# Algomorph/LevelSetFusion-Python

Measured on AMD Instinct MI355X. Metric: voxel-warp-updates/sec, higher is better.
Workload: dtype f32

## Files before the change

include/lsf_hip.h:

```cpp
#ifndef LSF_HIP_H
#define LSF_HIP_H

#include <stdint.h>

#ifdef __cplusplus
extern "C" {
#endif

#define LSF_ABI_VERSION 4
#define LSF_MAX_KERNEL_TAPS 31

#define LSF_ERR_BAD_ARGUMENT (-1)
#define LSF_ERR_BAD_DIMS (-2)
#define LSF_ERR_KERNEL_TOO_LONG (-3)
#define LSF_ERR_RCCL_UNAVAILABLE (-4)
#define LSF_ERR_RCCL_FAILED (-5)
#define LSF_ERR_NOT_RESIDENT (-6)

typedef struct lsf_grid {
    int32_t dims;
    int32_t nz, ny, nx;
    int32_t z_begin, z_end;
    int32_t z_global_offset;
    int32_t y_global_offset;
// ... 83 lines not shown
    int32_t previous_max;
    int32_t reserved;
    int32_t packed_nz;
    int32_t packed_z_global_offset;
} lsf_hier_params;

int lsf_hier_iteration(const float *packed_live4, const float *canonical, float *warp_planar,
                       const float *g_prev_planar, float *g_out_planar, const lsf_grid *grid,
                       const lsf_hier_params *params, const lsf_gate *gate, lsf_iteration_record *record,
                       void *stream);

int lsf_hier_level_run_2d(const float *packed_live4, const float *canonical, float *warp_a, float *warp_b, float *g_a,
                          float *g_b, const lsf_grid *grid, const lsf_hier_params *params, const double *taps_host,
                          int32_t n_taps, lsf_iteration_record *records, int32_t iterations,
                          int32_t iterations_per_launch, float threshold, void *stream);
int lsf_hier_update(const float *g_planar, float *warp_planar, const lsf_grid *grid, float rate,
                    const lsf_gate *gate, lsf_iteration_record *record, void *stream);

#define LSF_SMOOTHING_TIKHONOV 0
#define LSF_SMOOTHING_KILLING 1
#define LSF_DATA_BASIC 0
#define LSF_DATA_THRESHOLDED_FDM 2
#define LSF_ENERGY_NONE 0
#define LSF_ENERGY_DIRECT 1
#define LSF_ENERGY_VECTORIZED 2

typedef struct lsf_slavcheva_params {
    double isomorphic_enforcement_factor_f64;
    float rate;
    float data_term_weight;
    float smoothing_term_weight;
    float level_set_term_weight;
    float isomorphic_enforcement_factor;
    float killing_c1;
    int32_t smoothing_method;
    int32_t data_method;
    int32_t level_set_enabled;
    int32_t energy_mode;
    int32_t zero_gradient_on_snap;
    int32_t reserved;
} lsf_slavcheva_params;

int lsf_slavcheva_gradient(const float *live, const float *canonical, const float *warp_prev_planar,
                           float *g_out_planar, const lsf_grid *grid, const lsf_slavcheva_params *params,
                           const lsf_gate *gate, lsf_iteration_record *record, const int32_t *band_list,
                           int64_t band_count, void *stream);

#define LSF_BAND_ALL 0
#define LSF_BAND_INTERIOR 1
#define LSF_BAND_BOUNDARY 2

int64_t lsf_band_scratch_elements(const lsf_grid *grid);
int lsf_band_count(const float *live, const float *canonical, const lsf_grid *grid, int32_t subset,
                   int32_t *scratch, int64_t *count_out, void *stream);
int lsf_band_list_fill(const float *live, const float *canonical, const lsf_grid *grid, int32_t subset,
                       const int32_t *scratch, int32_t *list, void *stream);

int64_t lsf_state_prepare_scratch_elements(const lsf_grid *grid);
int lsf_state_pack_needed(const float *live, float *state_a, float *state_b, const lsf_grid *grid, int32_t *scratch,
                          int32_t reach, int32_t invert, void *stream);

int lsf_band_list_fill_prepared(const lsf_grid *grid, int32_t subset, const int32_t *scratch, int32_t *list,
                                void *stream);
int lsf_state_prepare(const float *live, const float *canonical, float *state_a, float *state_b,
                      const lsf_grid *grid, int32_t *scratch, int64_t *counts_out, void *stream);
int lsf_state_pack(const float *live, const float *warp_planar, float *state_a, float *state_b,
                   const lsf_grid *grid, void *stream);
int lsf_state_unpack(const float *state, float *live_out, float *warp_planar_out, float *warp_interleaved_out,
                     const lsf_grid *grid, void *stream);
int64_t lsf_state_finalize_scratch_elements(const lsf_grid *grid);
int lsf_state_finalize(const float *state, const float *canonical, float *live_out, float *warp_planar_out,
                       float *warp_interleaved_out, const lsf_grid *grid, float lower_threshold,
                       double *statistics16, double *scratch, void *stream);
int lsf_planar_finalize(const float *live, const float *warp_planar, const float *canonical, float *live_out,
                        float *warp_interleaved_out, const lsf_grid *grid, float lower_threshold,
                        double *statistics16, double *scratch, void *stream);

int lsf_state_finalize_listed(const float *state, const float *canonical, float *live_out, float *warp_interleaved_out,
                              const lsf_grid *grid, const int32_t *const *band_lists, const int64_t *band_counts,
                              int32_t n_lists, int64_t opposite_count, int64_t first_opposite, float lower_threshold,
                              double *statistics16, double *scratch, const int32_t *skip_flag,
                              const lsf_iteration_record *guard_records, int32_t guard_count, float guard_limit,
                              void *stream);
int lsf_slavcheva_state_iteration(const float *state_in, const float *canonical, float *state_out,
                                  const lsf_grid *grid, const lsf_slavcheva_params *params, const lsf_gate *gate,
                                  lsf_iteration_record *record, const int32_t *band_list, int64_t band_count,
                                  int32_t band_subset, void *stream);

int lsf_cumulative_warp_compose(const float *state, const float *psi_in, float *psi_out, const lsf_grid *grid,
                                const lsf_gate *gate, const int32_t *band_list, int64_t band_count, void *stream);

typedef struct lsf_band_box {
    int32_t origin;
    int32_t reserved;
    uint64_t mask;
} lsf_band_box;
int64_t lsf_band_boxes_scratch_elements(const lsf_grid *grid);
int lsf_band_boxes_count(const lsf_grid *grid, int32_t subset, const int32_t *prepare_scratch, int32_t *box_scratch,
                         int64_t *count_out, void *stream);
int lsf_band_boxes_fill(const lsf_grid *grid, int32_t subset, const int32_t *prepare_scratch, const int32_t *box_scratch,
                        lsf_band_box *boxes, void *stream);
int lsf_band_boxes_canonical(const float *canonical, const lsf_grid *grid, const lsf_band_box *boxes, int64_t box_count,
                             float *canonical_boxed, void *stream);
int lsf_slavcheva_state_iteration_boxes(const float *state_in, const float *canonical_boxed, float *state_out,
                                        const lsf_grid *grid, const lsf_slavcheva_params *params, const lsf_gate *gate,
                                        lsf_iteration_record *record, const lsf_band_box *boxes, int64_t box_count,
                                        void *stream);

typedef struct lsf_run_loop {
    int32_t min_iterations;
    int32_t max_iterations;
    float lower_threshold, upper_threshold;
    int32_t check_interval;
    int32_t reserved;
} lsf_run_loop;
typedef struct lsf_state_run {
    const float *live;
    const float *canonical;
    float *state[2];
    int32_t *prepare_scratch;
    int64_t *totals_device;
    int64_t *totals_host;
    lsf_grid grid;
    int32_t sparse_reach;
    int32_t second_state_late;
    int32_t *box_scratch;
    int32_t box_all;
    int32_t reserved;
} lsf_state_run;
typedef struct lsf_state_run_result {
    float *max_value;
    int64_t *argmax;
    double *energies3;
    uint8_t *executed;
    int32_t final_state;
    int32_t n_lists;
    int32_t reach_exceeded;
    int32_t compact_faces;
} lsf_state_run_result;
int lsf_state_run_begin(const lsf_state_run *run, void *stream);
int lsf_state_run_finish(const lsf_state_run *run, const lsf_slavcheva_params *params, int32_t *list_interior,
                         int32_t *list_boundary, lsf_band_box *boxes, float *box_canonical, lsf_iteration_record *records,
                         int32_t iterations, const lsf_run_loop *loop ,
                         float *live_out,
                         float lower_threshold, double *statistics16, double *finalize_scratch, int64_t *words_device,
                         int64_t *words_host, lsf_state_run_result *result, void *stream);
int lsf_state_run_finish_rows(const lsf_state_run *run, const lsf_slavcheva_params *params, int32_t *list_interior,
                              int32_t *list_boundary, lsf_band_box *boxes, float *box_canonical,
                              lsf_iteration_record *records, int32_t iterations, const lsf_run_loop *loop, float *live_out,
                              float lower_threshold, double *statistics16, double *finalize_scratch, int64_t *words_device,
                              int64_t *words_host, lsf_state_run_result *result, int64_t *record_rows,
                              int64_t record_rows_elements, int32_t *rows_taken, void *stream);
int64_t lsf_state_run_rows_elements(const lsf_grid *grid, int32_t iterations, int32_t n_lists);

int lsf_sobolev_run_finish(const lsf_state_run *run, const lsf_slavcheva_params *params, const double *taps_host,
                           int32_t n_taps, int32_t *list_interior, int32_t *list_boundary, int32_t *list_all,
                           lsf_band_box *boxes, float *g4_a, float *g4_b, lsf_iteration_record *records, int32_t iterations,
                           const lsf_run_loop *loop, float *live_out, float lower_threshold, double *statistics16,
                           double *finalize_scratch, int64_t *words_device, int64_t *words_host,
                           lsf_state_run_result *result, void *stream);

int lsf_sobolev_state_gradient(const float *state, const float *canonical, float *g_raw4, const lsf_grid *grid,
                               const lsf_slavcheva_params *params, const lsf_gate *gate, lsf_iteration_record *record,
                               const int32_t *band_list, int64_t band_count, void *stream);
int lsf_sobolev_state_gradient_x(const float *state, const float *canonical, float *out4, const lsf_grid *grid,
                                 const lsf_slavcheva_params *params, const double *taps_host, int32_t n_taps,
                                 const lsf_gate *gate, lsf_iteration_record *record, const int32_t *band_list,
                                 int64_t band_count, int32_t out_bricks, void *stream);
int lsf_zero_listed4(float *field4, const lsf_grid *grid, const int32_t *band_list, int64_t band_count, int32_t bricks,
                     void *stream);
int lsf_convolve_axis_listed4(const float *in4, float *out4, const float *zero_mask_source4, const lsf_grid *grid,
                              int32_t axis, const double *taps_host, int32_t n_taps, const lsf_gate *gate,
                              const int32_t *band_list, int64_t band_count, void *stream);
int lsf_band_list_strip_major(const int32_t *band_list, int64_t band_count, const lsf_grid *grid, int32_t strips,
                              int32_t *out, int32_t *scratch, void *stream);
int lsf_sobolev_state_update(const float *in4, const float *zero_mask_source4, const float *state_in, float *state_out,
                             float *g_out4, const lsf_grid *grid, const lsf_slavcheva_params *params, int32_t axis,
                             const double *taps_host, int32_t n_taps, const lsf_gate *gate,
                             lsf_iteration_record *record, const int32_t *band_list, int64_t band_count,
                             int32_t first_list, void *stream);
int lsf_sobolev_state_update_boxes(const float *in4, const float *state_in, float *state_out, float *g_out4,
                                   const lsf_grid *grid, const lsf_slavcheva_params *params, const double *taps_host,
                                   int32_t n_taps, const lsf_gate *gate, lsf_iteration_record *record,
                                   const lsf_band_box *boxes, int64_t box_count, void *stream);

#define LSF_SLAB_LAUNCH 0
#define LSF_SLAB_EXCHANGE 1
#define LSF_SLAB_EXCHANGE_DEFERRED 2
#define LSF_SLAB_RESUME 3
typedef struct lsf_slab_comm lsf_slab_comm;
typedef struct lsf_slab_layout {
    int32_t nz, ny, nx;
    int32_t z_begin, z_end;
    int32_t halo;
    int32_t lo_rank, hi_rank;
} lsf_slab_layout;
typedef struct lsf_slab_part {
    lsf_grid grid;
    const int32_t *band_list[2];
    int64_t band_count[2];
    int32_t band_subset[2];
    int32_t n_lists;
    int32_t reserved;
} lsf_slab_part;
typedef struct lsf_slab_faces {
    const int32_t *send_list[2], *recv_list[2];
    float *send_msg[2], *recv_msg[2];
    int64_t send_count[2], recv_count[2];
} lsf_slab_faces;
int lsf_merge_sorted_runs(const int32_t *const *a, const int64_t *n_a, const int32_t *const *b, const int64_t *n_b,
                          int32_t *const *out, int32_t pairs, void *stream);
int lsf_slab_unique_id(const char *rccl_library_path, uint8_t *id_out128);
int lsf_slab_comm_create(const char *rccl_library_path, const uint8_t *id128, int32_t rank, int32_t world,
                         lsf_slab_comm **out);
int lsf_slab_comm_destroy(lsf_slab_comm *comm);
int lsf_slab_comm_info(lsf_slab_comm *comm, int32_t *rank_out, int32_t *nranks_out);
int lsf_slab_face_counts_begin(lsf_slab_comm *comm, const int64_t *counts4);
int lsf_slab_face_counts_end(lsf_slab_comm *comm, int64_t *table);
int lsf_slab_state_iteration(lsf_slab_comm *comm, const float *state_in, const float *canonical, float *state_out,
                             const lsf_slab_layout *layout, const lsf_slab_part *boundary_parts, int32_t n_boundary,
                             const lsf_slab_part *interior_parts, int32_t n_interior,
                             const lsf_slavcheva_params *params, const lsf_gate *gate, lsf_iteration_record *record,
                             int32_t exchange ,
                             const lsf_slab_faces *faces , void *stream);

#define LSF_SLAB_MAX_CUTS 72
typedef struct lsf_slab_run {
    lsf_state_run base;
    lsf_slab_layout layout;
    int32_t exchange_interval;
    int32_t n_cuts;
    int32_t cut_slices[LSF_SLAB_MAX_CUTS];
    int64_t cut_entries[2][LSF_SLAB_MAX_CUTS];
    int64_t out_index_entries;
    int64_t out_face_entries;
} lsf_slab_run;
int lsf_slab_run_begin(lsf_slab_run *run, void *stream);
int lsf_slab_run_finish(const lsf_slab_run *run, lsf_slab_comm *comm, const lsf_slavcheva_params *params,
                        int32_t *list_interior, int32_t *list_boundary, int32_t *index_scratch, float *face_messages,
                        lsf_iteration_record *records, int32_t iterations, float *live_out, int64_t *words_device,
                        int64_t *words_host, lsf_state_run_result *result, void *stream);

int lsf_slavcheva_filter_update_rewarp(const float *in_planar, const float *zero_mask_source, const float *live,
                                       float *g_out_planar, float *warp_out_planar, float *live_out,
                                       const lsf_grid *grid, const lsf_slavcheva_params *params, int32_t axis,
                                       const double *taps_host, int32_t n_taps, const lsf_gate *gate,
                                       lsf_iteration_record *record, const int32_t *band_list, int64_t band_count,
                                       void *stream);

int lsf_slavcheva_update_rewarp(const float *live, const float *canonical, float *g_planar ,
                                float *warp_out_planar, float *live_out, const lsf_grid *grid,
                                const lsf_slavcheva_params *params, const lsf_gate *gate,
                                lsf_iteration_record *record, const int32_t *band_list ,
                                int64_t band_count, void *stream);

#define LSF_TERM_DATA_BASIC 0
#define LSF_TERM_DATA_THRESHOLDED_FDM 1
#define LSF_TERM_TIKHONOV 2
#define LSF_TERM_TIKHONOV_LOCAL 3
#define LSF_TERM_KILLING 4
#define LSF_TERM_LEVEL_SET 5
#define LSF_TERM_COPY_IF_ZERO 1
#define LSF_TERM_IGNORE_IF_ZERO 2
#define LSF_TERM_INTERLEAVED 4
#define LSF_SELECT_ALL 0
#define LSF_SELECT_BAND 1
#define LSF_SELECT_LIST 2
#define LSF_TERM_ENERGY_LOCAL 0
#define LSF_TERM_ENERGY_NP_GRADIENT 1

typedef struct lsf_term_params {
    double isomorphic_enforcement_factor_f64;
    float isomorphic_enforcement_factor;
    float epsilon;
    float scaling_factor;
    int32_t term;
    int32_t flags;
    int32_t reserved;
} lsf_term_params;

int lsf_term_gradient(const float *live, const float *canonical, const float *live_gradient_x,
                      const float *live_gradient_y, const float *live_gradient_z, const float *warp,
                      float *gradient_out, double *energy_out, double *energy_total, const lsf_grid *grid,
                      const lsf_term_params *params, int32_t selection, int32_t energy_form, const int32_t *indices,
                      int64_t index_count, void *stream);

int lsf_warp_statistics(const float *warp_planar, const float *canonical, const float *live,
                        const lsf_grid *grid, float lower_threshold, double *out8, void *stream);
int lsf_tsdf_difference_statistics(const float *canonical, const float *live, const lsf_grid *grid,
                                   double *out8, void *stream);

typedef struct lsf_tsdf_params {
    double intrinsics[4];
    double depth_unit_ratio;
    double voxel_size;
    double narrow_band_half_width;
    float extrinsic[16];
    int32_t array_offset[3];
    int32_t image_width, image_height;
    int32_t image_y_coordinate;
    float default_value;
    int32_t intrinsics_are_f32;
} lsf_tsdf_params;

int lsf_tsdf_generate_nearest(const uint16_t *depth_image, float *field, const lsf_grid *grid,
                              const lsf_tsdf_params *params, void *stream);
// ... 490 lines not shown
```

levelsetfusion-python_amd/_lib.py:

```python
import ctypes
import os

import torch

from ._build import LIB_PATH

c_float_p = ctypes.c_void_p

MAX_KERNEL_TAPS = 31
ABI_VERSION = 4
HEADER_ABI_HASH = "7b9c31a7c45631ef"

ERRORS = {-1: "LSF_ERR_BAD_ARGUMENT", -2: "LSF_ERR_BAD_DIMS", -3: "LSF_ERR_KERNEL_TOO_LONG",
          -4: "LSF_ERR_RCCL_UNAVAILABLE", -5: "LSF_ERR_RCCL_FAILED", -6: "LSF_ERR_NOT_RESIDENT"}

SMOOTHING_TIKHONOV, SMOOTHING_KILLING = 0, 1
DATA_BASIC, DATA_THRESHOLDED_FDM = 0, 2
ENERGY_NONE, ENERGY_DIRECT, ENERGY_VECTORIZED = 0, 1, 2
GATE_HIERARCHICAL, GATE_SLAVCHEVA, GATE_OPEN = 0, 1, 2


class Grid(ctypes.Structure):
    _fields_ = [("dims", ctypes.c_int32), ("nz", ctypes.c_int32), ("ny", ctypes.c_int32), ("nx", ctypes.c_int32),
                ("z_begin", ctypes.c_int32), ("z_end", ctypes.c_int32), ("z_global_offset", ctypes.c_int32),
                ("y_global_offset", ctypes.c_int32), ("energy_z_begin", ctypes.c_int32), ("energy_z_end", ctypes.c_int32),
                ("ny_global", ctypes.c_int32), ("energy_y_begin", ctypes.c_int32), ("energy_y_end", ctypes.c_int32)]


BAND_ALL, BAND_INTERIOR, BAND_BOUNDARY = 0, 1, 2
RECORD_SLOTS = 8


class RecordSlot(ctypes.Structure):
    _fields_ = [("max_packed", ctypes.c_uint64), ("data_energy", ctypes.c_double),
                ("smoothing_energy", ctypes.c_double), ("level_set_energy", ctypes.c_double),
                ("pad", ctypes.c_uint64 * 508)]


class IterationRecord(ctypes.Structure):
    _fields_ = [("slot", RecordSlot * RECORD_SLOTS)]


RECORD_BYTES = ctypes.sizeof(IterationRecord)
SLOT_WORDS = ctypes.sizeof(RecordSlot) // 8


class Gate(ctypes.Structure):
    _fields_ = [("prev_record", ctypes.c_void_p), ("mode", ctypes.c_int32), ("a", ctypes.c_float),
                ("b", ctypes.c_float)]


SLAB_LAUNCH, SLAB_EXCHANGE, SLAB_EXCHANGE_DEFERRED, SLAB_RESUME = 0, 1, 2, 3


class SlabLayoutC(ctypes.Structure):
    _fields_ = [("nz", ctypes.c_int32), ("ny", ctypes.c_int32), ("nx", ctypes.c_int32), ("z_begin", ctypes.c_int32),
                ("z_end", ctypes.c_int32), ("halo", ctypes.c_int32), ("lo_rank", ctypes.c_int32),
                ("hi_rank", ctypes.c_int32)]


class SlabPart(ctypes.Structure):
    _fields_ = [("grid", Grid), ("band_list", ctypes.c_void_p * 2), ("band_count", ctypes.c_int64 * 2),
                ("band_subset", ctypes.c_int32 * 2), ("n_lists", ctypes.c_int32), ("reserved", ctypes.c_int32)]


class SlabFaces(ctypes.Structure):
    _fields_ = [("send_list", ctypes.c_void_p * 2), ("recv_list", ctypes.c_void_p * 2),
                ("send_msg", ctypes.c_void_p * 2), ("recv_msg", ctypes.c_void_p * 2),
                ("send_count", ctypes.c_int64 * 2), ("recv_count", ctypes.c_int64 * 2)]


class BandBox(ctypes.Structure):
    _fields_ = [("origin", ctypes.c_int32), ("reserved", ctypes.c_int32), ("mask", ctypes.c_uint64)]


class StateRun(ctypes.Structure):
    _fields_ = [("live", ctypes.c_void_p), ("canonical", ctypes.c_void_p), ("state", ctypes.c_void_p * 2),
                ("prepare_scratch", ctypes.c_void_p), ("totals_device", ctypes.c_void_p),
                ("totals_host", ctypes.c_void_p), ("grid", Grid), ("sparse_reach", ctypes.c_int32),
                ("second_state_late", ctypes.c_int32), ("box_scratch", ctypes.c_void_p), ("box_all", ctypes.c_int32),
                ("reserved", ctypes.c_int32)]


TERM_DATA_BASIC, TERM_DATA_THRESHOLDED_FDM, TERM_TIKHONOV, TERM_TIKHONOV_LOCAL, TERM_KILLING, TERM_LEVEL_SET = range(6)
TERM_COPY_IF_ZERO, TERM_IGNORE_IF_ZERO, TERM_INTERLEAVED = 1, 2, 4
SELECT_ALL, SELECT_BAND, SELECT_LIST = 0, 1, 2
TERM_ENERGY_LOCAL, TERM_ENERGY_NP_GRADIENT = 0, 1


class TermParams(ctypes.Structure):
    _fields_ = [("isomorphic_enforcement_factor_f64", ctypes.c_double), ("isomorphic_enforcement_factor", ctypes.c_float),
                ("epsilon", ctypes.c_float), ("scaling_factor", ctypes.c_float), ("term", ctypes.c_int32),
                ("flags", ctypes.c_int32), ("reserved", ctypes.c_int32)]


class StateRunResult(ctypes.Structure):
    _fields_ = [("max_value", ctypes.c_void_p), ("argmax", ctypes.c_void_p), ("energies3", ctypes.c_void_p),
                ("executed", ctypes.c_void_p), ("final_state", ctypes.c_int32), ("n_lists", ctypes.c_int32),
                ("reach_exceeded", ctypes.c_int32), ("compact_faces", ctypes.c_int32)]


class RunLoop(ctypes.Structure):
    _fields_ = [("min_iterations", ctypes.c_int32), ("max_iterations", ctypes.c_int32), ("lower_threshold", ctypes.c_float),
                ("upper_threshold", ctypes.c_float), ("check_interval", ctypes.c_int32), ("reserved", ctypes.c_int32)]


SLAB_MAX_CUTS = 72


class SlabRun(ctypes.Structure):
    _fields_ = [("base", StateRun), ("layout", SlabLayoutC), ("exchange_interval", ctypes.c_int32),
                ("n_cuts", ctypes.c_int32), ("cut_slices", ctypes.c_int32 * SLAB_MAX_CUTS),
                ("cut_entries", (ctypes.c_int64 * SLAB_MAX_CUTS) * 2), ("out_index_entries", ctypes.c_int64),
                ("out_face_entries", ctypes.c_int64)]


class HierParams(ctypes.Structure):
    _fields_ = [("data_term_amplifier", ctypes.c_float), ("tikhonov_strength", ctypes.c_float),
                ("rate", ctypes.c_float), ("tikhonov_enabled", ctypes.c_int32), ("apply_update", ctypes.c_int32),
                ("compute_energy", ctypes.c_int32), ("previous_max", ctypes.c_int32), ("reserved", ctypes.c_int32),
                ("packed_nz", ctypes.c_int32), ("packed_z_global_offset", ctypes.c_int32)]


class SlavchevaParams(ctypes.Structure):
    _fields_ = [("isomorphic_enforcement_factor_f64", ctypes.c_double), ("rate", ctypes.c_float),
                ("data_term_weight", ctypes.c_float), ("smoothing_term_weight", ctypes.c_float),
                ("level_set_term_weight", ctypes.c_float), ("isomorphic_enforcement_factor", ctypes.c_float),
                ("killing_c1", ctypes.c_float), ("smoothing_method", ctypes.c_int32),
                ("data_method", ctypes.c_int32), ("level_set_enabled", ctypes.c_int32),
                ("energy_mode", ctypes.c_int32), ("zero_gradient_on_snap", ctypes.c_int32),
                ("reserved", ctypes.c_int32)]


class TsdfParams(ctypes.Structure):
    _fields_ = [("intrinsics", ctypes.c_double * 4), ("depth_unit_ratio", ctypes.c_double),
                ("voxel_size", ctypes.c_double), ("narrow_band_half_width", ctypes.c_double),
                ("extrinsic", ctypes.c_float * 16), ("array_offset", ctypes.c_int32 * 3),
                ("image_width", ctypes.c_int32), ("image_height", ctypes.c_int32),
                ("image_y_coordinate", ctypes.c_int32), ("default_value", ctypes.c_float),
                ("intrinsics_are_f32", ctypes.c_int32)]


DEPTH_U16, DEPTH_F32, DEPTH_F64 = 0, 1, 2
RIGID_RECORD_DOUBLES = 24
RIGID_MAX_BLOCKS = 256
RIGID_SCRATCH_BYTES = 2 * RIGID_MAX_BLOCKS * 10 * 8


class RigidParams(ctypes.Structure):
    _fields_ = [("tsdf", TsdfParams), ("array_offset", ctypes.c_double * 3), ("voxel_size", ctypes.c_double),
                ("twist", ctypes.c_double * 3),
                ("rate", ctypes.c_double), ("eta", ctypes.c_float), ("depth_dtype", ctypes.c_int32),
                ("height", ctypes.c_int32), ("width", ctypes.c_int32), ("iterations", ctypes.c_int32),
                ("reserved", ctypes.c_int32)]


RIGID3D_RECORD_DOUBLES = 64
RIGID3D_MAX_BLOCKS = 256
RIGID3D_SCRATCH_BYTES = 2 * RIGID3D_MAX_BLOCKS * 28 * 8


class Rigid3dParams(ctypes.Structure):
    _fields_ = [("tsdf", TsdfParams), ("array_offset", ctypes.c_double * 3), ("voxel_size", ctypes.c_double),
                ("twist", ctypes.c_double * 6),
                ("rate", ctypes.c_double), ("eta", ctypes.c_float), ("depth_dtype", ctypes.c_int32),
                ("depth", ctypes.c_int32), ("height", ctypes.c_int32), ("width", ctypes.c_int32),
                ("iterations", ctypes.c_int32)]
# ... 121 lines not shown


PYRAMID_MAX_RADIUS = 8
ICP_PYRAMID_SCRATCH_BYTES = 2 * ICP_MAX_BLOCKS * 30 * 8


class DepthPyramidParams(ctypes.Structure):
    _fields_ = [(n, ctypes.c_double) for n in ("fx", "fy", "cx", "cy", "depth_unit_ratio", "sigma_space",
                                               "sigma_range", "depth_gate")] + \
               [(n, ctypes.c_int32) for n in ("height", "width", "depth_dtype", "levels", "radius")]


class IcpPyramidParams(ctypes.Structure):
    _fields_ = [(n, ctypes.c_double) for n in ("fx", "fy", "cx", "cy", "max_distance", "cos_max_angle")] + \
               [("twist_p", ctypes.c_double * 6)] + \
               [(n, ctypes.c_int32) for n in ("height", "width", "pyramid_levels", "levels", "angle_gate")] + \
               [("iterations", ctypes.c_int32 * ICP_MAX_LEVELS)]


ICP_PHOTOMETRIC_SCRATCH_BYTES = 2 * ICP_MAX_BLOCKS * 31 * 8


class IcpPhotometricParams(ctypes.Structure):
    _fields_ = [(n, ctypes.c_double) for n in ("fx", "fy", "cx", "cy", "depth_unit_ratio", "max_distance",
                                               "photometric_weight", "max_intensity_difference")] + \
               [("twist_p", ctypes.c_double * 6)] + \
               [(n, ctypes.c_int32) for n in ("height", "width", "depth_dtype", "levels")] + \
               [("iterations", ctypes.c_int32 * ICP_MAX_LEVELS), ("strides", ctypes.c_int32 * ICP_MAX_LEVELS)]


INTENSITY_SOURCE_COLOUR, INTENSITY_SOURCE_PREDICTION = 0, 1


class IntensityPyramidParams(ctypes.Structure):
    _fields_ = [(n, ctypes.c_int32) for n in ("height", "width", "levels", "source")]


ICP_PYRAMID_PHOTOMETRIC_SCRATCH_BYTES = 2 * ICP_MAX_BLOCKS * 32 * 8


class IcpPyramidPhotometricParams(ctypes.Structure):
    _fields_ = [(n, ctypes.c_double) for n in ("fx", "fy", "cx", "cy", "max_distance", "cos_max_angle",
                                               "photometric_weight", "max_intensity_difference")] + \
               [("twist_p", ctypes.c_double * 6)] + \
               [(n, ctypes.c_int32) for n in ("height", "width", "pyramid_levels", "levels", "angle_gate",
                                              "reserved")] + \
               [("iterations", ctypes.c_int32 * ICP_MAX_LEVELS)]


ICP_LOSS_HUBER, ICP_LOSS_TUKEY = 1, 2
ICP_ROBUST_SCRATCH_BYTES = 2 * ICP_MAX_BLOCKS * 34 * 8
ICP_PYRAMID_ROBUST_SCRATCH_BYTES = 2 * ICP_MAX_BLOCKS * 35 * 8
_ROBUST_FIELDS = [("loss", ctypes.c_int32), ("scale", ctypes.c_double), ("intensity_scale", ctypes.c_double)]


class IcpRobustParams(ctypes.Structure):
    _fields_ = IcpPhotometricParams._fields_ + _ROBUST_FIELDS


class IcpPyramidRobustParams(ctypes.Structure):
    _fields_ = IcpPyramidPhotometricParams._fields_ + _ROBUST_FIELDS


POINT_SDF_LOSS_NONE = 0
POINT_SDF_SCRATCH_BYTES = 2 * ICP_MAX_BLOCKS * 33 * 8


class PointSdfParams(ctypes.Structure):
    _fields_ = [(n, ctypes.c_double) for n in ("fx", "fy", "cx", "cy", "depth_unit_ratio", "max_distance", "voxel_size",
                                               "offset_x", "offset_y", "offset_z", "narrow_band_width_voxels",
                                               "scale")] + \
               [(n, ctypes.c_int32) for n in ("depth", "height", "width", "image_height", "image_width", "depth_dtype",
                                              "levels")] + \
               [("iterations", ctypes.c_int32 * ICP_MAX_LEVELS), ("strides", ctypes.c_int32 * ICP_MAX_LEVELS),
                ("loss", ctypes.c_int32)]


POINT_SDF_COLOUR_SCRATCH_BYTES = 2 * ICP_MAX_BLOCKS * 35 * 8
_POINT_SDF_COLOUR_FIELDS = [(n, ctypes.c_double) for n in ("photometric_weight", "max_intensity_difference",
                                                           "intensity_scale")]


class PointSdfPhotometricParams(ctypes.Structure):
    _fields_ = PointSdfParams._fields_ + _POINT_SDF_COLOUR_FIELDS


class PointSdfPyramidParams(ctypes.Structure):
    _fields_ = PointSdfPhotometricParams._fields_ + [("pyramid_levels", ctypes.c_int32), ("reserved", ctypes.c_int32)]


class EwaParams(ctypes.Structure):
    _fields_ = [("covariance_camera_space", ctypes.c_double * 9), ("squared_radius_threshold", ctypes.c_double),
                ("intrinsic_matrix", ctypes.c_float * 9), ("method", ctypes.c_int32)]


_P = ctypes.POINTER
_vp, _i32, _i64, _f32 = ctypes.c_void_p, ctypes.c_int32, ctypes.c_int64, ctypes.c_float

PROTOTYPES = {
    "lsf_abi_version": (ctypes.c_int, []),
    "lsf_target_arch": (ctypes.c_char_p, []),
    "lsf_build_id": (ctypes.c_char_p, []),
    "lsf_abi_hash": (ctypes.c_char_p, []),
    "lsf_deinterleave": (ctypes.c_int, [_vp, _vp, _i64, _i32, _vp]),
    "lsf_interleave": (ctypes.c_int, [_vp, _vp, _i64, _i32, _vp]),
    "lsf_halo_copy": (ctypes.c_int, [_vp, _vp, _vp, _vp, _P(Grid), _i32, _i32, _i32, _i32, _i32, _vp]),
    "lsf_warp_field": (ctypes.c_int, [_vp, _vp, _vp, _P(Grid), _f32, _vp]),
    "lsf_warp_field_advanced": (ctypes.c_int, [_vp, _vp, _vp, _vp, _vp, _P(Grid), _i32, _vp]),
    "lsf_pack_live_gradient": (ctypes.c_int, [_vp, _vp, _P(Grid), _vp]),
    "lsf_restrict_mean": (ctypes.c_int, [_vp, _vp, _P(Grid), _i32, _vp]),
    "lsf_prolong_repeat": (ctypes.c_int, [_vp, _vp, _P(Grid), _vp]),
    "lsf_upsample2x_linear": (ctypes.c_int, [_vp, _vp, _P(Grid), _i32, _vp]),
    "lsf_downsample2x_linear": (ctypes.c_int, [_vp, _vp, _P(Grid), _i32, _vp]),
    "lsf_convolve_axis": (ctypes.c_int, [_vp, _vp, _vp, _P(Grid), _i32, _i32, _P(ctypes.c_double), _i32,
                                         _P(Gate), _vp]),
    "lsf_convolve_xy": (ctypes.c_int, [_vp, _vp, _P(Grid), _i32, _P(ctypes.c_double), _i32, _P(Gate), _vp]),
    "lsf_convolve_axis_update": (ctypes.c_int, [_vp, _vp, _vp, ctypes.c_float, _P(Grid), _i32, _i32, _P(ctypes.c_double),
                                                _i32, _P(Gate), _vp]),
    "lsf_convolve_xyz": (ctypes.c_int, [_vp, _vp, _vp, _f32, _P(Grid), _i32, _P(ctypes.c_double), _i32, _P(Gate),
                                        _vp]),
    "lsf_hier_iteration": (ctypes.c_int, [_vp, _vp, _vp, _vp, _vp, _P(Grid), _P(HierParams), _P(Gate), _vp, _vp]),
    "lsf_hier_update": (ctypes.c_int, [_vp, _vp, _P(Grid), _f32, _P(Gate), _vp, _vp]),
    "lsf_hier_level_run_2d": (ctypes.c_int, [_vp, _vp, _vp, _vp, _vp, _vp, _P(Grid), _P(HierParams), _P(ctypes.c_double),
                                            _i32, _vp, _i32, _i32, ctypes.c_float, _vp]),
    "lsf_slavcheva_gradient": (ctypes.c_int, [_vp, _vp, _vp, _vp, _P(Grid), _P(SlavchevaParams), _P(Gate), _vp,
                                              _vp, _i64, _vp]),
    "lsf_convolve_axis_listed": (ctypes.c_int, [_vp, _vp, _vp, _P(Grid), _i32, _i32, _P(ctypes.c_double), _i32,
                                                _P(Gate), _vp, _i64, _vp]),
    "lsf_state_prepare_scratch_elements": (ctypes.c_int64, [_P(Grid)]),
    "lsf_band_list_fill_prepared": (ctypes.c_int, [_P(Grid), _i32, _vp, _vp, _vp]),
    "lsf_state_prepare": (ctypes.c_int, [_vp, _vp, _vp, _vp, _P(Grid), _vp, _vp, _vp]),
    "lsf_state_pack": (ctypes.c_int, [_vp, _vp, _vp, _vp, _P(Grid), _vp]),
    "lsf_state_pack_needed": (ctypes.c_int, [_vp, _vp, _vp, _P(Grid), _vp, _i32, _i32, _vp]),
    "lsf_state_unpack": (ctypes.c_int, [_vp, _vp, _vp, _vp, _P(Grid), _vp]),
    "lsf_state_finalize_scratch_elements": (ctypes.c_int64, [_P(Grid)]),
    "lsf_state_finalize": (ctypes.c_int, [_vp, _vp, _vp, _vp, _vp, _P(Grid), _f32, _vp, _vp, _vp]),
    "lsf_planar_finalize": (ctypes.c_int, [_vp, _vp, _vp, _vp, _vp, _P(Grid), _f32, _vp, _vp, _vp]),
    "lsf_state_finalize_listed": (ctypes.c_int, [_vp, _vp, _vp, _vp, _P(Grid), _P(ctypes.c_void_p), _P(_i64), _i32,
                                                 _i64, _i64, _f32, _vp, _vp, _vp, _vp, _i32, _f32, _vp]),
    "lsf_slavcheva_state_iteration": (ctypes.c_int, [_vp, _vp, _vp, _P(Grid), _P(SlavchevaParams), _P(Gate), _vp,
                                                     _vp, _i64, _i32, _vp]),
    "lsf_cumulative_warp_compose": (ctypes.c_int, [_vp, _vp, _vp, _P(Grid), _P(Gate), _vp, _i64, _vp]),
    "lsf_band_boxes_scratch_elements": (ctypes.c_int64, [_P(Grid)]),
    "lsf_band_boxes_count": (ctypes.c_int, [_P(Grid), ctypes.c_int32, _vp, _vp, _vp, _vp]),
    "lsf_band_boxes_fill": (ctypes.c_int, [_P(Grid), ctypes.c_int32, _vp, _vp, _vp, _vp]),
    "lsf_band_boxes_canonical": (ctypes.c_int, [_vp, _P(Grid), _vp, ctypes.c_int64, _vp, _vp]),
    "lsf_slavcheva_state_iteration_boxes": (ctypes.c_int, [_vp, _vp, _vp, _P(Grid), _P(SlavchevaParams), _P(Gate), _vp, _vp,
                                                           _i64, _vp]),
    "lsf_state_run_begin": (ctypes.c_int, [_P(StateRun), _vp]),
    "lsf_state_run_finish_rows": (ctypes.c_int, [_P(StateRun), _P(SlavchevaParams), _vp, _vp, _vp, _vp, _vp, _i32, _P(RunLoop),
                                                 _vp, _f32, _vp, _vp, _vp, _vp, _P(StateRunResult), _vp, ctypes.c_int64,
                                                 _P(ctypes.c_int32), _vp]),
    "lsf_state_run_rows_elements": (ctypes.c_int64, [_P(Grid), _i32, _i32]),
    "lsf_state_run_finish": (ctypes.c_int, [_P(StateRun), _P(SlavchevaParams), _vp, _vp, _vp, _vp, _vp, _i32, _P(RunLoop), _vp,
                                            _f32, _vp, _vp, _vp, _vp, _P(StateRunResult), _vp]),
    "lsf_sobolev_run_finish": (ctypes.c_int, [_P(StateRun), _P(SlavchevaParams), _P(ctypes.c_double), _i32, _vp, _vp, _vp, _vp,
                                              _vp, _vp, _vp, _i32, _P(RunLoop), _vp, _f32, _vp, _vp, _vp, _vp,
                                              _P(StateRunResult), _vp]),
    "lsf_slab_run_begin": (ctypes.c_int, [_P(SlabRun), _vp]),
    "lsf_slab_run_finish": (ctypes.c_int, [_P(SlabRun), _vp, _P(SlavchevaParams), _vp, _vp, _vp, _vp, _vp, _i32, _vp, _vp, _vp,
                                           _P(StateRunResult), _vp]),
    "lsf_band_scratch_elements": (ctypes.c_int64, [_P(Grid)]),
    "lsf_band_count": (ctypes.c_int, [_vp, _vp, _P(Grid), _i32, _vp, _vp, _vp]),
    "lsf_band_list_fill": (ctypes.c_int, [_vp, _vp, _P(Grid), _i32, _vp, _vp, _vp]),
    "lsf_records_decode": (ctypes.c_int, [_vp, _i32, _i32, _i32, _vp, _vp, _vp, _vp]),
    "lsf_merge_sorted_runs": (ctypes.c_int, [_P(_vp), _P(_i64), _P(_vp), _P(_i64), _P(_vp), _i32, _vp]),
    "lsf_slab_unique_id": (ctypes.c_int, [ctypes.c_char_p, _vp]),
    "lsf_slab_comm_create": (ctypes.c_int, [ctypes.c_char_p, _vp, _i32, _i32, _P(_vp)]),
    "lsf_slab_comm_destroy": (ctypes.c_int, [_vp]),
    "lsf_slab_comm_info": (ctypes.c_int, [_vp, _P(_i32), _P(_i32)]),
    "lsf_slab_face_counts_begin": (ctypes.c_int, [_vp, _P(_i64)]),
    "lsf_slab_face_counts_end": (ctypes.c_int, [_vp, _P(_i64)]),
    "lsf_slab_state_iteration": (ctypes.c_int, [_vp, _vp, _vp, _vp, _P(SlabLayoutC), _P(SlabPart), _i32, _P(SlabPart),
                                                _i32, _P(SlavchevaParams), _P(Gate), _vp, _i32, _P(SlabFaces), _vp]),
    "lsf_slavcheva_filter_update_rewarp": (ctypes.c_int, [_vp, _vp, _vp, _vp, _vp, _vp, _P(Grid), _P(SlavchevaParams),
                                                          _i32, _P(ctypes.c_double), _i32, _P(Gate), _vp, _vp, _i64,
                                                          _vp]),
    "lsf_sobolev_state_gradient": (ctypes.c_int, [_vp, _vp, _vp, _P(Grid), _P(SlavchevaParams), _P(Gate), _vp, _vp, _i64,
                                                  _vp]),
    "lsf_band_list_strip_major": (ctypes.c_int, [_vp, _i64, _P(Grid), _i32, _vp, _vp, _vp]),
    "lsf_sobolev_state_gradient_x": (ctypes.c_int, [_vp, _vp, _vp, _P(Grid), _P(SlavchevaParams), _P(ctypes.c_double), _i32,
                                                    _P(Gate), _vp, _vp, _i64, _i32, _vp]),
    "lsf_zero_listed4": (ctypes.c_int, [_vp, _P(Grid), _vp, _i64, _i32, _vp]),
    "lsf_convolve_axis_listed4": (ctypes.c_int, [_vp, _vp, _vp, _P(Grid), _i32, _P(ctypes.c_double), _i32, _P(Gate), _vp,
                                                 _i64, _vp]),
    "lsf_sobolev_state_update": (ctypes.c_int, [_vp, _vp, _vp, _vp, _vp, _P(Grid), _P(SlavchevaParams), _i32,
                                                _P(ctypes.c_double), _i32, _P(Gate), _vp, _vp, _i64, _i32, _vp]),
    "lsf_sobolev_state_update_boxes": (ctypes.c_int, [_vp, _vp, _vp, _vp, _P(Grid), _P(SlavchevaParams),
                                                      _P(ctypes.c_double), _i32, _P(Gate), _vp, _vp, _i64, _vp]),
    "lsf_slavcheva_update_rewarp": (ctypes.c_int, [_vp, _vp, _vp, _vp, _vp, _P(Grid), _P(SlavchevaParams),
                                                   _P(Gate), _vp, _vp, _i64, _vp]),
    "lsf_term_gradient": (ctypes.c_int, [_vp, _vp, _vp, _vp, _vp, _vp, _vp, _vp, _vp, _P(Grid), _P(TermParams), _i32, _i32,
                                         _vp, _i64, _vp]),
    "lsf_warp_statistics": (ctypes.c_int, [_vp, _vp, _vp, _P(Grid), _f32, _vp, _vp]),
    "lsf_tsdf_difference_statistics": (ctypes.c_int, [_vp, _vp, _P(Grid), _vp, _vp]),
    "lsf_tsdf_generate_nearest": (ctypes.c_int, [_vp, _vp, _P(Grid), _P(TsdfParams), _vp]),
    "lsf_tsdf_generate_bilinear": (ctypes.c_int, [_vp, _vp, _P(Grid), _P(TsdfParams), _i32, _vp]),
    "lsf_tsdf_generate_ewa": (ctypes.c_int, [_vp, _vp, _P(Grid), _P(TsdfParams), _P(EwaParams), _vp]),
    "lsf_tsdf_generate_nearest_typed": (ctypes.c_int, [_vp, _i32, _vp, _P(Grid), _P(TsdfParams), _P(ctypes.c_double),
                                                       _P(ctypes.c_double), _vp]),
    "lsf_rigid_gradient": (ctypes.c_int, [_vp, _vp, _P(RigidParams), _vp]),
    "lsf_rigid_run": (ctypes.c_int, [_vp, _vp, _vp, _vp, _vp, _P(RigidParams), _vp]),
    "lsf_rigid3d_gradient": (ctypes.c_int, [_vp, _vp, _vp, _vp, _P(Rigid3dParams), _vp]),
    "lsf_rigid3d_run": (ctypes.c_int, [_vp, _vp, _vp, _vp, _vp, _P(Rigid3dParams), _vp]),
    "lsf_fusion_integrate_volume": (ctypes.c_int, [_vp, _vp, _vp, _vp, _vp, _P(FusionParams), _vp]),
    "lsf_fusion_integrate_depth": (ctypes.c_int, [_vp, _vp, _vp, _vp, _vp, _P(FusionParams), _vp]),
    "lsf_fusion_integrate_depth_weighted": (ctypes.c_int, [_vp, _vp, _vp, _vp, _vp, _vp, _P(FusionWeightedParams),
                                                           _vp]),
    "lsf_fusion_integrate_depth_colour": (ctypes.c_int, [_vp, _vp, _vp, _vp, _vp, _vp, _vp, _vp,
                                                         _P(FusionColourParams), _vp]),
    "lsf_fusion_integrate_depth_warped": (ctypes.c_int, [_vp, _vp, _vp, _vp, _vp, _vp, _vp, _vp, _vp,
                                                         _P(FusionWarpedParams), _vp]),
    "lsf_depth_confidence": (ctypes.c_int, [_vp, _vp, _vp, _P(DepthConfidenceParams), _vp]),
    "lsf_raycast": (ctypes.c_int, [_vp, _vp, _vp, _vp, _vp, _vp, _P(RaycastParams), _vp]),
    "lsf_raycast_colour": (ctypes.c_int, [_vp, _vp, _vp, _vp, _vp, _vp, _vp, _vp, _P(RaycastParams), _vp]),
    "lsf_mesh_count": (ctypes.c_int, [_vp, _vp, _vp, _vp, _vp, _vp, _P(MeshParams), _vp]),
    "lsf_mesh_emit": (ctypes.c_int, [_vp, _vp, _vp, _vp, _vp, _vp, _vp, _vp, _vp, _i64, _i64, _P(MeshParams), _vp]),
    "lsf_mesh_vertex_colours": (ctypes.c_int, [_vp, _vp, _vp, _vp, _vp, _i64, ctypes.c_int32, ctypes.c_int32,
                                               ctypes.c_int32, _P(MeshParams), _vp]),
    "lsf_volume_shift": (ctypes.c_int, [_vp, _vp, _vp, _vp, _vp, _vp, _P(VolumeShiftParams), _vp]),
    "lsf_volume_bricks_count": (ctypes.c_int, [_vp, _vp, _vp, _vp, _P(VolumeBricksParams), _vp]),
    "lsf_volume_bricks_gather": (ctypes.c_int, [_vp, _vp, _vp, _vp, _vp, _i64, _vp, _vp, _vp, _vp, _vp,
                                                _P(VolumeBricksParams), _vp]),
    "lsf_volume_bricks_scatter": (ctypes.c_int, [_vp, _vp, _vp, _vp, _vp, _i64, _vp, _vp, _vp,
                                                 _P(VolumeBricksParams), _vp]),
    "lsf_rgbd_ray_table": (ctypes.c_int, [_vp, _vp, _P(RgbdParams), _vp]),
    "lsf_rgbd_register_depth": (ctypes.c_int, [_vp, ctypes.c_int32, _vp, _vp, _vp, _vp, _vp, _vp, _P(RgbdParams), _vp]),
    "lsf_rgbd_rectify_colour": (ctypes.c_int, [_vp, _vp, _vp, _P(RgbdParams), _vp]),
    "lsf_reloc_encode": (ctypes.c_int, [_vp, ctypes.c_int32, _vp, _vp, _vp, _vp, _P(RelocParams), _vp]),
    "lsf_reloc_query": (ctypes.c_int, [_vp] * 9 + [_P(RelocParams), _vp]),
    "lsf_icp_run": (ctypes.c_int, [_vp, _vp, _vp, _vp, _vp, _vp, _vp, _P(IcpParams), _vp]),
    "lsf_depth_pyramid": (ctypes.c_int, [_vp, _vp, _vp, _P(DepthPyramidParams), _vp]),
    "lsf_icp_run_pyramid": (ctypes.c_int, [_vp, _vp, _vp, _vp, _vp, _vp, _vp, _vp, _P(IcpPyramidParams), _vp]),
    "lsf_icp_run_photometric": (ctypes.c_int, [_vp, _vp, _vp, _vp, _vp, _vp, _vp, _vp, _vp, _vp,
                                               _P(IcpPhotometricParams), _vp]),
    "lsf_intensity_pyramid": (ctypes.c_int, [_vp, _vp, _P(IntensityPyramidParams), _vp]),
    "lsf_icp_run_pyramid_photometric": (ctypes.c_int, [_vp, _vp, _vp, _vp, _vp, _vp, _vp, _vp, _vp, _vp, _vp,
                                                       _P(IcpPyramidPhotometricParams), _vp]),
    "lsf_icp_run_robust": (ctypes.c_int, [_vp, _vp, _vp, _vp, _vp, _vp, _vp, _vp, _vp, _vp, _vp, _P(IcpRobustParams),
                                          _vp]),
    "lsf_icp_run_pyramid_robust": (ctypes.c_int, [_vp, _vp, _vp, _vp, _vp, _vp, _vp, _vp, _vp, _vp, _vp, _vp,
                                                  _P(IcpPyramidRobustParams), _vp]),
    "lsf_point_sdf_run": (ctypes.c_int, [_vp, _vp, _vp, _vp, _vp, _vp, _vp, _vp, _P(PointSdfParams), _vp]),
    "lsf_point_sdf_run_photometric": (ctypes.c_int, [_vp] * 11 + [_P(PointSdfPhotometricParams), _vp]),
    "lsf_point_sdf_run_pyramid": (ctypes.c_int, [_vp] * 11 + [_P(PointSdfPyramidParams), _vp]),
}


class LsfHipError(RuntimeError):
    pass


def _load():
    path = os.environ.get("LSF_HIP_LIBRARY") or LIB_PATH
    if not os.path.exists(path):
        raise ImportError(
            "liblsf_hip.so is missing (%s).  This package has no CPU fallback: build the HIP library first with\n"
            "    python -c 'import __graft_entry__ as g; g.build()'      (needs hipcc, cross-compiles gfx950)"
            % path)
    lib = ctypes.CDLL(path)
    for name, (restype, argtypes) in PROTOTYPES.items():
        if argtypes is None:
            continue
        fn = getattr(lib, name)
        fn.restype = restype
        fn.argtypes = argtypes
    if lib.lsf_abi_version() != ABI_VERSION:
        raise ImportError("liblsf_hip.so ABI version %d != binding version %d: rebuild" %
                          (lib.lsf_abi_version(), ABI_VERSION))
    built_against = lib.lsf_abi_hash().decode()
    if built_against != HEADER_ABI_HASH:
        raise ImportError("%s was compiled from an include/lsf_hip.h whose structures / prototypes hash to %s; this binding "
                          "was written against %s: rebuild the library (or update the binding to the header)"
                          % (path, built_against, HEADER_ABI_HASH))
    return lib


lib = _load()

def check(status, what):
    if status == 0:
        return
    if status in ERRORS:
        raise LsfHipError("%s: %s" % (what, ERRORS[status]))
    raise LsfHipError("%s: HIP error %d" % (what, status))
```

levelsetfusion-python_amd/csrc/lsf_device.h:

```cpp
#pragma once

#include <hip/hip_runtime.h>
#include <cstdlib>
#include <stdint.h>

#include "../../include/lsf_hip.h"

namespace lsf {

constexpr int kWave = 64;
constexpr int kBlock = 256;
constexpr int kCuBlock = 1024;
constexpr int kMaxBlockWaves = kCuBlock / kWave;

struct FastDiv {
    unsigned d, m, l;
};

__host__ inline FastDiv make_fast_div(unsigned d) {
    FastDiv f;
    f.d = d;
    f.l = 0;
    while ((1ull << f.l) < d) ++f.l;
    f.m = (unsigned)(((1ull << 32) * ((1ull << f.l) - d)) / d + 1ull);
// ... 435 lines not shown
#define LSF_STEP(CTRL)                                   \
    {                                                    \
        const unsigned long long o = dpp_u64<CTRL>(v);   \
        v = o > v ? o : v;                               \
    }
    LSF_DPP_STEPS(LSF_STEP)
#undef LSF_STEP
    return broadcast_lane63_u64(v);
}

__device__ inline double wave_sum_f64(double v) {
#define LSF_STEP(CTRL) v += dpp_f64<CTRL>(v);
    LSF_DPP_STEPS(LSF_STEP)
#undef LSF_STEP
    return __longlong_as_double((long long)broadcast_lane63_u64((unsigned long long)__double_as_longlong(v)));
}

__device__ inline unsigned long long pack_max(float length, unsigned linear_index) {
    return ((unsigned long long)__float_as_uint(length) << 32) | (unsigned long long)(~linear_index);
}

__device__ inline float unpack_max_value(unsigned long long packed) { return __uint_as_float((unsigned)(packed >> 32)); }

template <int NS>
__device__ inline void block_reduce_commit(unsigned long long packed, const double (&sums)[NS > 0 ? NS : 1],
                                           unsigned long long* dst_max, double* const (&dst_sum)[NS > 0 ? NS : 1]) {
    __shared__ unsigned long long s_max[kMaxBlockWaves];
    __shared__ double s_sum[(NS > 0 ? NS : 1)][kMaxBlockWaves];
    const int lane = threadIdx.x & (kWave - 1), wave = threadIdx.x / kWave;
    const int n_waves = blockDim.x / kWave;
    unsigned long long m = wave_max_u64(packed);
    double s[NS > 0 ? NS : 1];
#pragma unroll
    for (int i = 0; i < NS; ++i) s[i] = wave_sum_f64(sums[i]);
    if (lane == 0) {
        s_max[wave] = m;
#pragma unroll
        for (int i = 0; i < NS; ++i) s_sum[i][wave] = s[i];
    }
    __syncthreads();
    if (wave == 0) {
        const unsigned long long mm = wave_max_u64(lane < n_waves ? s_max[lane] : 0ull);
        double t[NS > 0 ? NS : 1];
#pragma unroll
        for (int i = 0; i < NS; ++i) t[i] = wave_sum_f64(lane < n_waves ? s_sum[i][lane] : 0.0);
        if (lane == 0) {
            if (dst_max && mm != 0ull) atomicMax(dst_max, mm);
#pragma unroll
            for (int i = 0; i < NS; ++i)
                if (dst_sum[i] && t[i] != 0.0) atomicAdd(dst_sum[i], t[i]);
        }
    }
}

struct alignas(32) RecordRow {
    unsigned long long max_packed;
    double data, smoothing, level_set;
};

__device__ inline void wave_reduce_store_row(unsigned long long packed, const double (&sums)[3], RecordRow* __restrict__ rows) {
    RecordRow r;
    r.max_packed = packed;
    r.data = sums[0];
    r.smoothing = sums[1];
    r.level_set = sums[2];
#define LSF_STEP(CTRL)                                                                                             \
    {                                                                                                              \
        const unsigned long long om = dpp_u64<CTRL>(r.max_packed);                                                 \
        const double o0 = dpp_f64<CTRL>(r.data), o1 = dpp_f64<CTRL>(r.smoothing), o2 = dpp_f64<CTRL>(r.level_set); \
        r.max_packed = om > r.max_packed ? om : r.max_packed;                                                      \
        r.data += o0;                                                                                              \
        r.smoothing += o1;                                                                                         \
        r.level_set += o2;                                                                                         \
    }
    LSF_DPP_STEPS(LSF_STEP)
#undef LSF_STEP
    if ((threadIdx.x & (kWave - 1)) == kWave - 1) rows[blockIdx.x * (blockDim.x / kWave) + threadIdx.x / kWave] = r;
}

__host__ inline unsigned launch_rows(unsigned blocks, unsigned threads) { return blocks * (threads / kWave); }

template <int NT>
struct TapsN {
    double k[NT];
};

template <bool FMA>
__device__ inline double mac(double acc, double k, double v) {
    return FMA ? __builtin_fma(k, v, acc) : acc + k * v;
}

static inline bool taps_are_float32(const double* taps, int n) {
    for (int j = 0; j < n; ++j)
        if (!((double)(float)taps[j] == taps[j])) return false;
    return true;
}

template <int D>
__device__ inline float vec_length(const float (&v)[3]) {
    float s = v[0] * v[0] + v[1] * v[1];
    if (D == 3) s = s + v[2] * v[2];
    return sqrtf(s);
}

__device__ inline float second_difference_f64(float am, float a0, float ap) {
    return (float)__builtin_fma(-2.0, (double)a0, (double)ap + (double)am);
}

__device__ inline bool gate_closed(const lsf_gate& gate) {
    if (!gate.prev_record || gate.mode == LSF_GATE_OPEN) return false;
    unsigned long long p = 0ull;
#pragma unroll
    for (int k = 0; k < LSF_RECORD_SLOTS; ++k) {
        const unsigned long long q = gate.prev_record->slot[k].max_packed;
        p = q > p ? q : p;
    }
    if (p == 0ull) return true;
    float m = unpack_max_value(p);
    if (gate.mode == LSF_GATE_HIERARCHICAL) return m < gate.a;
    return !(gate.a < m && m < gate.b);
}

__device__ inline lsf_record_slot* record_slot(lsf_iteration_record* r) {
    return &r->slot[blockIdx.x % LSF_RECORD_SLOTS];
}

__device__ inline unsigned long long* record_max(lsf_iteration_record* r) {
    return reinterpret_cast<unsigned long long*>(&record_slot(r)->max_packed);
}

__host__ inline lsf_gate gate_or_open(const lsf_gate* gate) {
    return gate ? *gate : lsf_gate{nullptr, 0, 0.0f, 0.0f};
}

inline bool overlaps(const void* a, size_t na, const void* b, size_t nb) {
    if (!a || !b || !na || !nb) return false;
    const uintptr_t x = (uintptr_t)a, y = (uintptr_t)b;
    return x < y + nb && y < x + na;
}

inline hipStream_t as_stream(void* s) { return reinterpret_cast<hipStream_t>(s); }

inline int launch_status() { return (int)hipGetLastError(); }

int state_iteration_launch(const float* state_in, const float* canonical, float* state_out, const lsf_grid* grid,
                           const lsf_slavcheva_params* params, const lsf_gate* gate, lsf_iteration_record* record,
                           const int32_t* band_list, int64_t band_count, int32_t band_subset, RecordRow* rows,
                           unsigned rows_capacity, unsigned* rows_written, void* stream);
int state_iteration_boxes_launch(const float* state_in, const float* canonical_boxed, float* state_out, const lsf_grid* grid,
                                 const lsf_slavcheva_params* params, const lsf_gate* gate, lsf_iteration_record* record,
                                 const lsf_band_box* boxes, int64_t box_count, RecordRow* rows, unsigned rows_capacity,
                                 unsigned* rows_written, void* stream);
int state_prepare_launch(const float* live, const float* canonical, float* state_a, float* state_b, const lsf_grid* grid,
                         int32_t* scratch, int64_t* counts_out, bool zero_fifth, void* stream);
unsigned state_iteration_rows_max(const lsf_grid* grid);
unsigned state_iteration_boxes_rows_max(const lsf_grid* grid);
int state_finalize_listed_launch(const float* state, const float* canonical, float* live_out, float* warp_interleaved_out,
                                 const lsf_grid* grid, const int32_t* const* band_lists, const int64_t* band_counts,
                                 int32_t n_lists, int64_t opposite_count, int64_t first_opposite, float lower_threshold,
                                 double* statistics16, double* scratch, const int32_t* skip_flag,
                                 const lsf_iteration_record* guard_records, int32_t guard_count, float guard_limit,
                                 const lsf_iteration_record* word_records, int32_t n_word_slots, int64_t* words_out,
                                 void* stream);

}
```

levelsetfusion-python_amd/csrc/lsf_slavcheva.hip:

```cpp
#include "lsf_device.h"

using namespace lsf;

#include "lsf_slavcheva_terms.h"

using namespace lsf::slav;

namespace {


template <int D, int SMOOTH, bool LEVELSET, int DATA, int ENERGY>
__device__ inline void voxel_gradient(const float* __restrict__ live, const float* __restrict__ canonical,
                                      const float* __restrict__ warp_prev, const Grid& g, const Params& p, int x,
                                      int y, int z, int i, float (&gv)[3], double (&en)[3]) {
    gv[0] = gv[1] = gv[2] = 0.0f;
    const float l = live[i], cn = canonical[i];
    if (fabsf(l) == 1.0f && fabsf(cn) == 1.0f) return;
    const bool interior = x > 0 && x < g.nx - 1 && y > 0 && y < g.ny - 1 && (D == 2 || (z > 0 && z < g.nz - 1));
    if (g.fast_ok && __all(interior)) {
        const NbhFast<D> n(live, warp_prev, g, x, y, z);
        band_voxel_gradient<D, SMOOTH, LEVELSET, DATA, ENERGY>(n, p, l, cn, gv, en);
    } else {
        const Nbh<D> n(live, warp_prev, g, x, y, z);
        band_voxel_gradient<D, SMOOTH, LEVELSET, DATA, ENERGY>(n, p, l, cn, gv, en);
// ... 230 lines not shown
#pragma unroll
    for (int j = 0; j < 4; ++j) {
        const unsigned v = blockIdx.x * kBandChunk + j * kBlock + t;
        bool in_band = false;
        if (v < n) in_band = !(fabsf(live[first + v]) == 1.0f && fabsf(canonical[first + v]) == 1.0f);
        if (in_band && subset != LSF_BAND_ALL) {
            const unsigned i = first + v;
            const unsigned zy = fast_div(i, g.div_nx);
            const int x = (int)(i - zy * (unsigned)g.nx);
            const int z = (int)fast_div(zy, g.div_ny);
            const int y = (int)zy - z * g.ny;
            const bool interior = x > 0 && x < g.nx - 1 && y > 0 && y < g.ny - 1 && (dims == 2 || (z > 0 && z < g.nz - 1));
            in_band = interior == (subset == LSF_BAND_INTERIOR);
        }
        masks[j] = __ballot(in_band);
        if (lane == 0) part[j * 4 + wave] = __popcll(masks[j]);
    }
    __syncthreads();
    if (!FILL) {
        if (t == 0) {
            int sum = 0;
            for (int k = 0; k < 16; ++k) sum += part[k];
            block_sums[blockIdx.x] = sum;
        }
        return;
    }
    int at = block_sums[blockIdx.x];
#pragma unroll
    for (int j = 0; j < 4; ++j) {
#pragma unroll
        for (int wv = 0; wv < 4; ++wv) {
            if (wv == wave && ((masks[j] >> lane) & 1ull))
                list[at + __popcll(masks[j] & ((1ull << lane) - 1ull))] =
                    (int)(first + blockIdx.x * kBandChunk + j * kBlock + t);
            at += part[j * 4 + wv];
        }
    }
}

__device__ inline void reduce_opposite(const int* __restrict__ opposite, unsigned chunks, long long* __restrict__ totals) {
    __shared__ long long s_sum[1024 / kWave];
    __shared__ int s_first[1024 / kWave];
    long long sum = 0;
    int first = 0x7fffffff;
    for (unsigned c = threadIdx.x; c < chunks; c += 1024) {
        sum += opposite[2 * c];
        first = min(first, opposite[2 * c + 1]);
    }
    for (int d = kWave / 2; d > 0; d >>= 1) {
        sum += (long long)shfl_down_u64((unsigned long long)sum, d);
        first = min(first, __shfl_down(first, d, kWave));
    }
    if ((threadIdx.x & (kWave - 1)) == 0) {
        s_sum[threadIdx.x / kWave] = sum;
        s_first[threadIdx.x / kWave] = first;
    }
    __syncthreads();
    if (threadIdx.x == 0) {
        for (int k = 1; k < 1024 / kWave; ++k) {
            sum += s_sum[k];
            first = min(first, s_first[k]);
        }
        totals[2] = sum;
        totals[3] = first == 0x7fffffff ? -1 : first;
    }
}

__global__ __launch_bounds__(1024) void band_scan_kernel(int* __restrict__ sums_base, unsigned n, unsigned stride,
                                                         unsigned arrays, long long* totals,
                                                         const int* __restrict__ opposite) {
    if (blockIdx.x >= arrays) {
        reduce_opposite(opposite, n, totals);
        return;
    }
    __shared__ int wave_total[1024 / kWave];
    int* __restrict__ sums = sums_base + (size_t)blockIdx.x * stride;
    const unsigned t = threadIdx.x, lane = t & (kWave - 1), wave = t / kWave;
    int carry = 0;
    for (unsigned base = 0; base < n; base += 4096u) {
        const unsigned i = base + 4u * t;
        int v[4];
#pragma unroll
        for (int k = 0; k < 4; ++k) v[k] = i + k < n ? sums[i + k] : 0;
        const int mine = v[0] + v[1] + v[2] + v[3];
        int inclusive = mine;
#pragma unroll
        for (int d = 1; d < kWave; d <<= 1) {
            const int up = __shfl_up(inclusive, d, kWave);
            if ((int)lane >= d) inclusive += up;
        }
        if (lane == kWave - 1) wave_total[wave] = inclusive;
        __syncthreads();
        int before = 0, tile = 0;
#pragma unroll
        for (int w = 0; w < 1024 / kWave; ++w) {
            const int x = wave_total[w];
            before += w < (int)wave ? x : 0;
            tile += x;
        }
        int run = carry + before + inclusive - mine;
#pragma unroll
        for (int k = 0; k < 4; ++k) {
            if (i + k < n) sums[i + k] = run;
            run += v[k];
        }
        carry += tile;
        __syncthreads();
    }
    if (t == 0) totals[blockIdx.x] = carry;
}

constexpr unsigned kScanTile = 4096u;

__global__ __launch_bounds__(1024) void band_tile_totals_kernel(const int* __restrict__ sums_base, unsigned n,
                                                                unsigned stride, const int* __restrict__ opposite,
                                                                int* __restrict__ tile_out, unsigned tiles) {
    __shared__ int s_sum[1024 / kWave], s_first[1024 / kWave];
    const unsigned tile = blockIdx.x, a = blockIdx.y, t = threadIdx.x;
    const unsigned i = tile * kScanTile + 4u * t;
    int sum = 0, first = 0x7fffffff;
    if (a < 2u) {
        const int* __restrict__ sums = sums_base + (size_t)a * stride;
#pragma unroll
        for (unsigned k = 0; k < 4u; ++k) sum += i + k < n ? sums[i + k] : 0;
    } else {
#pragma unroll
        for (unsigned k = 0; k < 4u; ++k)
            if (i + k < n) {
                sum += opposite[2 * (i + k)];
                first = min(first, opposite[2 * (i + k) + 1]);
            }
    }
    for (int d = kWave / 2; d > 0; d >>= 1) {
        sum += __shfl_down(sum, d, kWave);
        first = min(first, __shfl_down(first, d, kWave));
    }
    if ((t & (kWave - 1)) == 0) {
        s_sum[t / kWave] = sum;
        s_first[t / kWave] = first;
    }
    __syncthreads();
    if (t == 0) {
        for (int k = 1; k < 1024 / kWave; ++k) {
            sum += s_sum[k];
            first = min(first, s_first[k]);
        }
        tile_out[(size_t)a * tiles + tile] = sum;
        if (a == 2u) tile_out[(size_t)3 * tiles + tile] = first;
    }
}

__global__ __launch_bounds__(1024) void band_scan_tiles_kernel(int* __restrict__ sums_base, unsigned n, unsigned stride,
                                                               const int* __restrict__ tile_out, unsigned tiles,
                                                               long long* __restrict__ totals, int zero_fifth) {
    const unsigned tile = blockIdx.x, a = blockIdx.y, t = threadIdx.x, lane = t & (kWave - 1), wave = t / kWave;
    if (a == 2u) {
        if (tile == 0u && t == 0u) {
            if (zero_fifth) totals[4] = 0;
            long long sum = 0;
            int first = 0x7fffffff;
            for (unsigned k = 0; k < tiles; ++k) {
                sum += tile_out[(size_t)2 * tiles + k];
                first = min(first, tile_out[(size_t)3 * tiles + k]);
            }
            totals[2] = sum;
            totals[3] = first == 0x7fffffff ? -1 : first;
        }
        return;
    }
    __shared__ int wave_total[1024 / kWave];
    int* __restrict__ sums = sums_base + (size_t)a * stride;
    int carry = 0;
    for (unsigned k = 0; k < tile; ++k) carry += tile_out[(size_t)a * tiles + k];
    const unsigned i = tile * kScanTile + 4u * t;
    int v[4];
#pragma unroll
    for (int k = 0; k < 4; ++k) v[k] = i + k < n ? sums[i + k] : 0;
    const int mine = v[0] + v[1] + v[2] + v[3];
    int inclusive = mine;
#pragma unroll
    for (int d = 1; d < kWave; d <<= 1) {
        const int up = __shfl_up(inclusive, d, kWave);
        if ((int)lane >= d) inclusive += up;
    }
    if (lane == kWave - 1) wave_total[wave] = inclusive;
    __syncthreads();
    int before = 0, whole = 0;
#pragma unroll
    for (int w = 0; w < 1024 / kWave; ++w) {
        const int x = wave_total[w];
        before += w < (int)wave ? x : 0;
        whole += x;
    }
    int run = carry + before + inclusive - mine;
#pragma unroll
    for (int k = 0; k < 4; ++k) {
        if (i + k < n) sums[i + k] = run;
        run += v[k];
    }
    if (tile == tiles - 1u && t == 0u) totals[a] = (long long)carry + whole;
}

typedef float vf4 __attribute__((ext_vector_type(4)));

__global__ __launch_bounds__(kBlock) void state_prepare_kernel(const float* __restrict__ live,
                                                               const float* __restrict__ canonical,
                                                               vf4* __restrict__ a, vf4* __restrict__ b, unsigned n,
                                                               Grid g, int dims, int* __restrict__ sums_interior,
                                                               int* __restrict__ sums_boundary,
                                                               unsigned long long* __restrict__ masks,
                                                               int* __restrict__ opposite, int* __restrict__ nonempty) {
    __shared__ int part[4][16];
    const int t = threadIdx.x, wave = t / kWave, lane = t % kWave;
#pragma unroll
    for (int j = 0; j < 4; ++j) {
        const unsigned v = blockIdx.x * kBandChunk + j * kBlock + t;
        bool in_band = false, interior = false, opposed = false;
        if (v < n) {
            const float l = live[v], cn = canonical[v];
            in_band = !(fabsf(l) == 1.0f && fabsf(cn) == 1.0f);
            opposed = !in_band && l != cn;
            vf4 o;
            o.x = l; o.y = 0.0f; o.z = 0.0f; o.w = 0.0f;
            if (a) a[v] = o;
            if (b) b[v] = o;
            const unsigned zy = fast_div(v, g.div_nx);
            const int x = (int)(v - zy * (unsigned)g.nx);
            const int z = (int)fast_div(zy, g.div_ny);
            const int y = (int)zy - z * g.ny;
            interior = x > 0 && x < g.nx - 1 && y > 0 && y < g.ny - 1 && (dims == 2 || (z > 0 && z < g.nz - 1));
        }
        const unsigned long long mi = __ballot(in_band && interior), mb = __ballot(in_band && !interior);
        const unsigned long long mo = __ballot(opposed);
        if (lane == 0) {
            part[0][j * 4 + wave] = __popcll(mi);
            part[1][j * 4 + wave] = __popcll(mb);
            part[2][j * 4 + wave] = __popcll(mo);
            part[3][j * 4 + wave] = mo ? (int)(blockIdx.x * kBandChunk + j * kBlock + wave * kWave) + __ffsll((long long)mo) - 1
                                       : 0x7fffffff;
            masks[((size_t)blockIdx.x * 16 + j * 4 + wave) * 2 + 0] = mi;
            masks[((size_t)blockIdx.x * 16 + j * 4 + wave) * 2 + 1] = mb;
        }
    }
    __syncthreads();
    if (t < 2) {
        int sum = 0;
        for (int k = 0; k < 16; ++k) sum += part[t][k];
        (t == 0 ? sums_interior : sums_boundary)[blockIdx.x] = sum;
    } else if (t == 2) {
        int sum = 0, first = 0x7fffffff;
        for (int k = 0; k < 16; ++k) {
            sum += part[2][k];
            first = min(first, part[3][k]);
        }
        opposite[2 * blockIdx.x] = sum;
        opposite[2 * blockIdx.x + 1] = first;
    } else if (t == 3) {
        int any = 0;
        for (int k = 0; k < 16; ++k) any |= part[0][k] | part[1][k];
        nonempty[blockIdx.x] = any != 0;
    }
}

constexpr int kPrepareChunksPerBlock = 4;
__device__ inline unsigned long long row16_or(unsigned nibble, int lane) {
    const int pos = lane & 15;
    unsigned lo = pos < 8 ? nibble << (4 * pos) : 0u, hi = pos < 8 ? 0u : nibble << (4 * (pos - 8));
#pragma unroll
    for (int d = 1; d < 16; d <<= 1) {
        lo |= (unsigned)__shfl_xor((int)lo, d, kWave);
        hi |= (unsigned)__shfl_xor((int)hi, d, kWave);
    }
    return ((unsigned long long)hi << 32) | lo;
}

__global__ __launch_bounds__(kBlock) void state_prepare4_kernel(const vf4* __restrict__ live4,
                                                                const vf4* __restrict__ canonical4,
                                                                vf4* __restrict__ a, vf4* __restrict__ b, unsigned n,
                                                                unsigned chunks, Grid g, int dims,
                                                                int* __restrict__ sums_interior,
                                                                int* __restrict__ sums_boundary,
                                                                unsigned long long* __restrict__ masks,
                                                                int* __restrict__ opposite, int* __restrict__ nonempty) {
    __shared__ int part[kPrepareChunksPerBlock][4][16];
    const int t = threadIdx.x, wave = t / kWave, lane = t % kWave;
    const unsigned chunk0 = blockIdx.x * kPrepareChunksPerBlock;
    vf4 l[kPrepareChunksPerBlock], c[kPrepareChunksPerBlock];
#pragma unroll
    for (int k = 0; k < kPrepareChunksPerBlock; ++k) {
        const unsigned v = (chunk0 + k) * kBandChunk + 4u * t;
        const vf4 one = {1.0f, 1.0f, 1.0f, 1.0f};
        l[k] = v < n ? live4[v / 4] : one;
        c[k] = v < n ? canonical4[v / 4] : one;
    }
#pragma unroll
    for (int k = 0; k < kPrepareChunksPerBlock; ++k) {
        const unsigned chunk = chunk0 + k, v = chunk * kBandChunk + 4u * t;
        unsigned ni = 0u, nb = 0u, no = 0u;
        if (v < n) {
            const unsigned zy = fast_div(v, g.div_nx);
            const int x0 = (int)(v - zy * (unsigned)g.nx);
            const int z = (int)fast_div(zy, g.div_ny);
            const int y = (int)zy - z * g.ny;
            const bool row_inside = y > 0 && y < g.ny - 1 && (dims == 2 || (z > 0 && z < g.nz - 1));
            const float lv[4] = {l[k].x, l[k].y, l[k].z, l[k].w}, cv[4] = {c[k].x, c[k].y, c[k].z, c[k].w};
#pragma unroll
            for (int j = 0; j < 4; ++j) {
                const bool in_band = !(fabsf(lv[j]) == 1.0f && fabsf(cv[j]) == 1.0f);
                const bool interior = row_inside && x0 + j > 0 && x0 + j < g.nx - 1;
                ni |= (in_band && interior ? 1u : 0u) << j;
                nb |= (in_band && !interior ? 1u : 0u) << j;
                no |= (!in_band && lv[j] != cv[j] ? 1u : 0u) << j;
                vf4 o;
                o.x = lv[j]; o.y = 0.0f; o.z = 0.0f; o.w = 0.0f;
                if (a) a[v + j] = o;
                if (b) b[v + j] = o;
            }
        }
        const unsigned long long mi = row16_or(ni, lane), mb = row16_or(nb, lane), mo = row16_or(no, lane);
        if ((lane & 15) == 0 && chunk < chunks) {
            const int word = wave * 4 + lane / 16;
            part[k][0][word] = __popcll(mi);
            part[k][1][word] = __popcll(mb);
            part[k][2][word] = __popcll(mo);
            part[k][3][word] = mo ? (int)(chunk * kBandChunk + word * kWave) + __ffsll((long long)mo) - 1 : 0x7fffffff;
            masks[((size_t)chunk * 16 + word) * 2 + 0] = mi;
            masks[((size_t)chunk * 16 + word) * 2 + 1] = mb;
        }
    }
    __syncthreads();
    if (t < 4 * kPrepareChunksPerBlock) {
        const int k = t / 4, what = t % 4;
        const unsigned chunk = chunk0 + k;
        if (chunk < chunks) {
            if (what < 2) {
                int sum = 0;
                for (int w = 0; w < 16; ++w) sum += part[k][what][w];
                (what == 0 ? sums_interior : sums_boundary)[chunk] = sum;
            } else if (what == 2) {
                int sum = 0, first = 0x7fffffff;
                for (int w = 0; w < 16; ++w) {
                    sum += part[k][2][w];
                    first = min(first, part[k][3][w]);
                }
                opposite[2 * chunk] = sum;
                opposite[2 * chunk + 1] = first;
            } else {
                int any = 0;
                for (int w = 0; w < 16; ++w) any |= part[k][0][w] | part[k][1][w];
                nonempty[chunk] = any != 0;
            }
        }
    }
}

__device__ inline bool chunk_is_needed(unsigned c, unsigned chunks, long long row, long long slice, int dims, int reach,
                                       const int* __restrict__ nonempty) {
    const int lane = threadIdx.x % kWave;
    const long long c0 = (long long)c * kBandChunk;
    const int span = 2 * reach + 1, zs = dims == 3 ? span : 1;
    bool hit = false;
    for (int k = lane; k < zs * span; k += kWave) {
        const int dy = k % span - reach, dz = dims == 3 ? k / span - reach : 0;
        const long long lo = c0 + dz * slice + dy * row - reach, hi = c0 + (long long)kBandChunk - 1 + dz * slice + dy * row + reach;
        long long first = lo >= 0 ? lo / kBandChunk : -((-lo + kBandChunk - 1) / kBandChunk);
        long long last = hi >= 0 ? hi / kBandChunk : -((-hi + kBandChunk - 1) / kBandChunk);
        first = first < 0 ? 0 : first;
        last = last >= (long long)chunks ? (long long)chunks - 1 : last;
        int flag[3];
#pragma unroll
        for (int j = 0; j < 3; ++j) flag[j] = first + j <= last ? nonempty[first + j] : 0;
        hit |= (flag[0] | flag[1] | flag[2]) != 0;
    }
    return __any(hit);
}

constexpr int kPackGroup = 32;
constexpr int kPackGroups = (int)kBandChunk / kPackGroup;
static_assert(kPackGroups == 32 && kWave == 2 * kPackGroups && kBlock % kPackGroups == 0,
              "a chunk's verdicts fill the int kept per chunk; two half waves per ballot");
__device__ inline unsigned group_verdicts_of_wave(unsigned c, unsigned chunks, long long row, long long slice, int dims,
                                                  int reach, const unsigned long long* __restrict__ masks) {
    const int span = 2 * reach + 1, offsets = span * (dims == 3 ? span : 1);
    const long long bits = (long long)chunks * kBandChunk;
    const long long g0 = (long long)c * kBandChunk + (threadIdx.x % kPackGroups) * kPackGroup;
    constexpr int kStep = kBlock / kPackGroups, kBatch = 4;
    bool hit = false;
    for (int k0 = threadIdx.x / kPackGroups; k0 < offsets; k0 += kBatch * kStep) {
        unsigned long long first[kBatch], second[kBatch], upto[kBatch];
        bool one[kBatch];
#pragma unroll
        for (int u = 0; u < kBatch; ++u) {
            const int k = k0 + u * kStep;
            const int dy = k % span - reach, dz = dims == 3 ? k / span - reach : 0;
            long long lo = g0 + dz * slice + dy * row - reach, hi = g0 + kPackGroup - 1 + dz * slice + dy * row + reach;
            lo = lo < 0 ? 0 : lo;
            hi = hi >= bits ? bits - 1 : hi;
            const bool inside = k < offsets && lo <= hi;
            const long long w0 = inside ? lo >> 6 : 0, w1 = inside ? hi >> 6 : 0;
            first[u] = (masks[2 * w0] | masks[2 * w0 + 1]) & (inside ? ~0ull << (lo & 63) : 0ull);
            second[u] = masks[2 * w1] | masks[2 * w1 + 1];
            upto[u] = ~0ull >> (63 - (hi & 63));
            one[u] = w0 == w1;
        }
#pragma unroll
        for (int u = 0; u < kBatch; ++u)
            hit |= (one[u] ? first[u] & upto[u] : first[u] | (second[u] & upto[u])) != 0ull;
    }
    const unsigned long long both = __ballot(hit);
    return (unsigned)both | (unsigned)(both >> 32);
}

__global__ __launch_bounds__(kBlock) void state_pack_needed_kernel(const float* __restrict__ live, vf4* __restrict__ a,
                                                                   vf4* __restrict__ b, unsigned n, unsigned chunks,
                                                                   int* __restrict__ needed, int want, int reach,
                                                                   long long row, long long slice, int dims,
                                                                   const int* __restrict__ nonempty,
                                                                   const unsigned long long* __restrict__ masks,
                                                                   int groups) {
    const int t = threadIdx.x;
    const unsigned c = blockIdx.x;
    __shared__ unsigned s_share[kBlock / kWave];
    unsigned mask;
    if (reach > 0) {
        if (!chunk_is_needed(c, chunks, row, slice, dims, reach, nonempty)) {
            if (t == 0) needed[c] = 0;
            return;
        }
        if (!groups) {
            if (t == 0) needed[c] = 1;
            mask = ~0u;
        } else {
            const unsigned share = group_verdicts_of_wave(c, chunks, row, slice, dims, reach, masks);
            if (t % kWave == 0) s_share[t / kWave] = share;
            __syncthreads();
            mask = 0u;
#pragma unroll
            for (int w = 0; w < kBlock / kWave; ++w) mask |= s_share[w];
            if (t == 0) needed[c] = (int)mask;
        }
    } else {
        mask = groups ? (unsigned)needed[c] : needed[c] != 0 ? ~0u : 0u;
    }
    if (want == 0) mask = ~mask;
    float l[4];
#pragma unroll
    for (int j = 0; j < 4; ++j) {
        const unsigned at = j * kBlock + t, v = c * kBandChunk + at;
        l[j] = ((mask >> (at / kPackGroup)) & 1u) != 0u && v < n ? live[v] : 0.0f;
    }
#pragma unroll
    for (int j = 0; j < 4; ++j) {
        const unsigned at = j * kBlock + t, v = c * kBandChunk + at;
        if (((mask >> (at / kPackGroup)) & 1u) != 0u && v < n) {
            vf4 o;
            o.x = l[j]; o.y = 0.0f; o.z = 0.0f; o.w = 0.0f;
            if (a) a[v] = o;
            if (b) b[v] = o;
        }
    }
}

__global__ __launch_bounds__(kBlock) void band_fill_from_masks_kernel(const unsigned long long* __restrict__ masks,
                                                                      const int* __restrict__ block_sums, int which,
                                                                      int* __restrict__ list, unsigned chunks) {
    const int lane = threadIdx.x % kWave;
    const unsigned chunk = blockIdx.x * (kBlock / kWave) + threadIdx.x / kWave;
    if (chunk >= chunks) return;
    const unsigned long long mine = lane < 16 ? masks[((size_t)chunk * 16 + lane) * 2 + which] : 0ull;
    if (__ballot(mine != 0ull) == 0ull) return;
    int at = block_sums[chunk];
#pragma unroll
    for (int w = 0; w < 16; ++w) {
        const unsigned lo = (unsigned)__shfl((int)(unsigned)mine, w, kWave);
        const unsigned hi = (unsigned)__shfl((int)(unsigned)(mine >> 32), w, kWave);
        const unsigned long long m = ((unsigned long long)hi << 32) | lo;
        if ((m >> lane) & 1ull)
            list[at + __popcll(m & ((1ull << lane) - 1ull))] = (int)(chunk * kBandChunk + w * kWave + lane);
        at += __popcll(m);
    }
}

}

static inline bool band_subset_ok(int32_t subset) {
    return subset == LSF_BAND_ALL || subset == LSF_BAND_INTERIOR || subset == LSF_BAND_BOUNDARY;
}

extern "C" int lsf_slavcheva_gradient(const float* live, const float* canonical, const float* warp_prev_planar,
                                      float* g_out_planar, const lsf_grid* grid, const lsf_slavcheva_params* params,
                                      const lsf_gate* gate, lsf_iteration_record* record, const int32_t* band_list,
                                      int64_t band_count, void* stream) {
    if (int e = check_grid(grid)) return e;
    if (!live || !canonical || !warp_prev_planar || !params || !record || !g_out_planar ||
        g_out_planar == warp_prev_planar || (band_list && (band_count < 0 || band_count > 0x7fffffffll)))
        return LSF_ERR_BAD_ARGUMENT;
    Grid g = make_grid(grid);
    Tiling t = make_tiling(g);
    if (t.total == 0) return 0;
    LaunchArgs a{band_list ? band_list_blocks((unsigned)band_count) : launch_blocks(t.total), as_stream(stream), live,
                 canonical, warp_prev_planar, g_out_planar, g, make_params(params), gate_or_open(gate), record, band_list,
                 (unsigned)band_count};
    if (grid->dims == 2) pick_terms<2>(params, a);
    else pick_terms<3>(params, a);
    return launch_status();
}

extern "C" int lsf_slavcheva_update_rewarp(const float* live, const float* canonical, float* g_planar,
                                           float* warp_out_planar, float* live_out, const lsf_grid* grid,
                                           const lsf_slavcheva_params* params, const lsf_gate* gate,
                                           lsf_iteration_record* record, const int32_t* band_list, int64_t band_count,
                                           void* stream) {
    (void)canonical;
    if (int e = check_grid(grid)) return e;
    if (!live || !g_planar || !warp_out_planar || !live_out || live_out == live || !params || !record ||
        (band_list && (band_count < 0 || band_count > 0x7fffffffll)))
        return LSF_ERR_BAD_ARGUMENT;
    Grid g = make_grid(grid);
    Tiling t = make_tiling(g);
    if (t.total == 0) return 0;
    Params p = make_params(params);
    lsf_gate gt = gate_or_open(gate);
    const unsigned blocks = band_list ? band_list_blocks((unsigned)band_count) : launch_blocks(t.total);
    if (grid->dims == 2)
        hipLaunchKernelGGL(slavcheva_update_rewarp_kernel<2>, dim3(blocks), dim3(kBlock), 0, as_stream(stream), live,
                           g_planar, warp_out_planar, live_out, g, p, gt, record, band_list, (unsigned)band_count);
    else
        hipLaunchKernelGGL(slavcheva_update_rewarp_kernel<3>, dim3(blocks), dim3(kBlock), 0, as_stream(stream), live,
                           g_planar, warp_out_planar, live_out, g, p, gt, record, band_list, (unsigned)band_count);
    return launch_status();
}

template <int D, int NT>
static void launch_filter_update(bool fma, unsigned blocks, hipStream_t s, const float* in, const float* mask,
                                 const float* live, float* g_out, float* warp_out, float* live_out, const Grid& g,
                                 const Params& p, const double* taps_host, int axis, const lsf_gate& gt,
                                 lsf_iteration_record* record, const int* list, unsigned count) {
    TapsN<NT> taps;
    for (int j = 0; j < NT; ++j) taps.k[j] = taps_host[j];
    if (fma)
        hipLaunchKernelGGL((slavcheva_filter_update_rewarp_kernel<D, NT, true>), dim3(blocks), dim3(kBlock), 0, s, in, mask,
                           live, g_out, warp_out, live_out, g, p, taps, axis, gt, record, list, count);
    else
        hipLaunchKernelGGL((slavcheva_filter_update_rewarp_kernel<D, NT, false>), dim3(blocks), dim3(kBlock), 0, s, in, mask,
                           live, g_out, warp_out, live_out, g, p, taps, axis, gt, record, list, count);
}

extern "C" int lsf_slavcheva_filter_update_rewarp(const float* in_planar, const float* zero_mask_source,
                                                  const float* live, float* g_out_planar, float* warp_out_planar,
                                                  float* live_out, const lsf_grid* grid,
                                                  const lsf_slavcheva_params* params, int32_t axis,
                                                  const double* taps_host, int32_t n_taps, const lsf_gate* gate,
                                                  lsf_iteration_record* record, const int32_t* band_list,
                                                  int64_t band_count, void* stream) {
    if (int e = check_grid(grid)) return e;
    if (!in_planar || !zero_mask_source || !live || !g_out_planar || !warp_out_planar || !live_out ||
        live_out == live || g_out_planar == in_planar || !params || !record || !taps_host || !band_list ||
        band_count < 0 || band_count > 0x7fffffffll || axis < 0 || axis >= grid->dims)
        return LSF_ERR_BAD_ARGUMENT;
    if (n_taps != 3 && n_taps != 5 && n_taps != 7 && n_taps != 9) return LSF_ERR_KERNEL_TOO_LONG;
    Grid g = make_grid(grid);
    if (g.z_end == g.z_begin) return 0;
    const Params p = make_params(params);
    const lsf_gate gt = gate_or_open(gate);
    const unsigned blocks = band_list_blocks((unsigned)band_count);
    hipStream_t s = as_stream(stream);
    bool fma = true;
    for (int j = 0; j < n_taps; ++j) fma = fma && (double)(float)taps_host[j] == taps_host[j];
    const int* list = band_list;
    const unsigned count = (unsigned)band_count;
#define LSF_FUR(D, NT) launch_filter_update<D, NT>(fma, blocks, s, in_planar, zero_mask_source, live, g_out_planar, \
                                                 warp_out_planar, live_out, g, p, taps_host, axis, gt, record, list, count)
    if (grid->dims == 2) {
        switch (n_taps) { case 3: LSF_FUR(2, 3); break; case 5: LSF_FUR(2, 5); break; case 7: LSF_FUR(2, 7); break; default: LSF_FUR(2, 9); break; }
    } else {
        switch (n_taps) { case 3: LSF_FUR(3, 3); break; case 5: LSF_FUR(3, 5); break; case 7: LSF_FUR(3, 7); break; default: LSF_FUR(3, 9); break; }
    }
#undef LSF_FUR
    return launch_status();
}

static inline bool band_range(const lsf_grid* grid, unsigned& first, unsigned& n, unsigned& chunks) {
    const long long slice = (long long)grid->ny * grid->nx;
    first = (unsigned)(slice * grid->z_begin);
    n = (unsigned)(slice * (grid->z_end - grid->z_begin));
    chunks = (n + kBandChunk - 1) / kBandChunk;
    return n > 0;
}

extern "C" int64_t lsf_band_scratch_elements(const lsf_grid* grid) {
    if (check_grid(grid)) return 0;
    unsigned first, n, chunks;
    band_range(grid, first, n, chunks);
    return (int64_t)chunks + 1;
}

extern "C" int lsf_band_count(const float* live, const float* canonical, const lsf_grid* grid, int32_t subset,
                              int32_t* scratch, int64_t* count_out, void* stream) {
    if (int e = check_grid(grid)) return e;
    if (!live || !canonical || !scratch || !count_out || !band_subset_ok(subset)) return LSF_ERR_BAD_ARGUMENT;
    unsigned first, n, chunks;
    band_range(grid, first, n, chunks);
    hipStream_t s = as_stream(stream);
    if (chunks > 0)
        hipLaunchKernelGGL(band_list_kernel<false>, dim3(chunks), dim3(kBlock), 0, s, live, canonical, first, n,
                           make_grid(grid), grid->dims, subset, scratch, (int*)nullptr);
    hipLaunchKernelGGL(band_scan_kernel, dim3(1), dim3(1024), 0, s, scratch, chunks, 0u, 1u, (long long*)count_out,
                       (const int*)nullptr);
    return launch_status();
}

static inline unsigned long long* prepare_masks(int32_t* scratch, unsigned chunks) {
    return reinterpret_cast<unsigned long long*>(scratch + 2 * (size_t)(chunks + 1) + (2 * (chunks + 1)) % 2);
}

static inline int* prepare_opposite(int32_t* scratch, unsigned chunks) {
    return reinterpret_cast<int*>(prepare_masks(scratch, chunks) + (size_t)chunks * 32);
}

static inline int* prepare_nonempty(int32_t* scratch, unsigned chunks) { return prepare_opposite(scratch, chunks) + 2 * (size_t)chunks; }
static inline int* prepare_needed(int32_t* scratch, unsigned chunks) { return prepare_nonempty(scratch, chunks) + chunks; }
static inline unsigned prepare_scan_tiles(unsigned chunks) { return (chunks + kScanTile - 1u) / kScanTile; }
static inline int* prepare_tile_totals(int32_t* scratch, unsigned chunks) { return prepare_needed(scratch, chunks) + chunks; }

extern "C" int64_t lsf_state_prepare_scratch_elements(const lsf_grid* grid) {
    if (check_grid(grid, true)) return 0;
    unsigned first, n, chunks;
    band_range(grid, first, n, chunks);
    return 2 * (int64_t)(chunks + 1) + 64 * (int64_t)chunks + 2 + 2 * (int64_t)chunks + 2 * (int64_t)chunks +
           4 * ((int64_t)prepare_scan_tiles(chunks) + 1);
}

extern "C" int lsf_band_list_fill_prepared(const lsf_grid* grid, int32_t subset, const int32_t* scratch, int32_t* list,
                                           void* stream) {
    if (int e = check_grid(grid, true)) return e;
    if (!scratch || !list || (subset != LSF_BAND_INTERIOR && subset != LSF_BAND_BOUNDARY) || grid->z_begin != 0 ||
        grid->z_end != grid->nz)
        return LSF_ERR_BAD_ARGUMENT;
    unsigned first, n, chunks;
    if (!band_range(grid, first, n, chunks)) return 0;
    const int which = subset == LSF_BAND_INTERIOR ? 0 : 1;
    hipLaunchKernelGGL(band_fill_from_masks_kernel, dim3((chunks + kBlock / kWave - 1) / (kBlock / kWave)), dim3(kBlock),
                       0, as_stream(stream), prepare_masks(const_cast<int32_t*>(scratch), chunks),
                       scratch + which * (size_t)(chunks + 1), which, list, chunks);
    return launch_status();
}

namespace {
constexpr int kBoxGroup = kBlock;

__device__ inline unsigned long long box_mask_of(const unsigned long long* __restrict__ masks, unsigned box, int nbx,
                                                 int nby, int nx, int ny, bool all) {
    const int bx = (int)(box % (unsigned)nbx), by = (int)((box / (unsigned)nbx) % (unsigned)nby);
    const int bz = (int)(box / ((unsigned)nbx * (unsigned)nby));
    unsigned long long m = 0ull;
#pragma unroll
    for (int k = 0; k < 4; ++k)
#pragma unroll
        for (int j = 0; j < 4; ++j) {
            const unsigned v = (unsigned)(((4 * bz + k) * ny + 4 * by + j) * nx + 4 * bx);
            const unsigned long long word = masks[2 * (size_t)(v >> 6)] | (all ? masks[2 * (size_t)(v >> 6) + 1] : 0ull);
            m |= ((word >> (v & 63u)) & 0xFull) << (4 * (k * 4 + j));
        }
    return m;
}

template <bool FILL>
__global__ __launch_bounds__(kBlock) void band_boxes_kernel(const unsigned long long* __restrict__ masks, unsigned n_boxes,
                                                            int nbx, int nby, int nx, int ny, bool all,
                                                            int* __restrict__ group_sums, lsf_band_box* __restrict__ boxes) {
    __shared__ int wave_count[kBlock / kWave];
    const unsigned box = blockIdx.x * kBoxGroup + threadIdx.x;
    const int lane = threadIdx.x % kWave, wave = threadIdx.x / kWave;
    const unsigned long long m = box < n_boxes ? box_mask_of(masks, box, nbx, nby, nx, ny, all) : 0ull;
    const unsigned long long any = __ballot(m != 0ull);
    if (lane == 0) wave_count[wave] = __popcll(any);
    __syncthreads();
    if (!FILL) {
        if (threadIdx.x == 0) {
            int sum = 0;
            for (int k = 0; k < kBlock / kWave; ++k) sum += wave_count[k];
            group_sums[blockIdx.x] = sum;
        }
        return;
    }
    if (m == 0ull) return;
    int at = group_sums[blockIdx.x];
    for (int k = 0; k < wave; ++k) at += wave_count[k];
    at += __popcll(any & ((1ull << lane) - 1ull));
    const int bx = (int)(box % (unsigned)nbx), by = (int)((box / (unsigned)nbx) % (unsigned)nby);
    const int bz = (int)(box / ((unsigned)nbx * (unsigned)nby));
    lsf_band_box b;
    b.origin = ((4 * bz) * ny + 4 * by) * nx + 4 * bx;
    b.reserved = 0;
    b.mask = m;
    boxes[at] = b;
}

inline bool boxes_ok(const lsf_grid* g) {
    return g->dims == 3 && g->nx % 4 == 0 && g->ny % 4 == 0 && g->nz % 4 == 0 && g->z_begin == 0 && g->z_end == g->nz &&
           (long long)g->nx * g->ny * g->nz <= 0x0fffffffll;
}
}

extern "C" int64_t lsf_band_boxes_scratch_elements(const lsf_grid* grid) {
    if (check_grid(grid) || !boxes_ok(grid)) return 0;
    const long long n_boxes = (long long)grid->nx * grid->ny * grid->nz / 64;
    return (n_boxes + kBoxGroup - 1) / kBoxGroup + 1;
}

extern "C" int lsf_band_boxes_count(const lsf_grid* grid, int32_t subset, const int32_t* prepare_scratch,
                                    int32_t* box_scratch, int64_t* count_out, void* stream) {
    if (int e = check_grid(grid)) return e;
    if (!boxes_ok(grid)) return LSF_ERR_BAD_DIMS;
    if (!prepare_scratch || !box_scratch || !count_out || (subset != LSF_BAND_INTERIOR && subset != LSF_BAND_ALL))
        return LSF_ERR_BAD_ARGUMENT;
    unsigned first, n, chunks;
    band_range(grid, first, n, chunks);
    const unsigned n_boxes = n / 64, groups = (n_boxes + kBoxGroup - 1) / kBoxGroup;
    hipStream_t s = as_stream(stream);
    hipLaunchKernelGGL(band_boxes_kernel<false>, dim3(groups), dim3(kBlock), 0, s,
                       prepare_masks(const_cast<int32_t*>(prepare_scratch), chunks), n_boxes, grid->nx / 4, grid->ny / 4,
                       grid->nx, grid->ny, subset == LSF_BAND_ALL, box_scratch, (lsf_band_box*)nullptr);
    hipLaunchKernelGGL(band_scan_kernel, dim3(1), dim3(1024), 0, s, box_scratch, groups, 0u, 1u, (long long*)count_out,
                       (const int*)nullptr);
    return launch_status();
}

extern "C" int lsf_band_boxes_fill(const lsf_grid* grid, int32_t subset, const int32_t* prepare_scratch,
                                   const int32_t* box_scratch, lsf_band_box* boxes, void* stream) {
    if (int e = check_grid(grid)) return e;
    if (!boxes_ok(grid)) return LSF_ERR_BAD_DIMS;
    if (!prepare_scratch || !box_scratch || !boxes || (subset != LSF_BAND_INTERIOR && subset != LSF_BAND_ALL))
        return LSF_ERR_BAD_ARGUMENT;
    unsigned first, n, chunks;
    band_range(grid, first, n, chunks);
    const unsigned n_boxes = n / 64, groups = (n_boxes + kBoxGroup - 1) / kBoxGroup;
    hipLaunchKernelGGL(band_boxes_kernel<true>, dim3(groups), dim3(kBlock), 0, as_stream(stream),
                       prepare_masks(const_cast<int32_t*>(prepare_scratch), chunks), n_boxes, grid->nx / 4, grid->ny / 4,
                       grid->nx, grid->ny, subset == LSF_BAND_ALL, const_cast<int32_t*>(box_scratch), boxes);
    return launch_status();
}

extern "C" int lsf_state_prepare(const float* live, const float* canonical, float* state_a, float* state_b,
                                 const lsf_grid* grid, int32_t* scratch, int64_t* counts_out, void* stream) {
    return state_prepare_launch(live, canonical, state_a, state_b, grid, scratch, counts_out, false, stream);
}

int lsf::state_prepare_launch(const float* live, const float* canonical, float* state_a, float* state_b, const lsf_grid* grid,
                              int32_t* scratch, int64_t* counts_out, bool zero_fifth, void* stream) {
    if (int e = check_grid(grid, true)) return e;
    if (!live || !canonical || (!state_a && state_b) || !scratch || !counts_out) return LSF_ERR_BAD_ARGUMENT;
    if (grid->z_begin != 0 || grid->z_end != grid->nz) return LSF_ERR_BAD_ARGUMENT;
    unsigned first, n, chunks;
    band_range(grid, first, n, chunks);
    hipStream_t s = as_stream(stream);
    int* sums_interior = scratch;
    int* sums_boundary = scratch + (chunks + 1);
    const bool wide = grid->nx % 4 == 0 && ((uintptr_t)live | (uintptr_t)canonical) % 16 == 0;
    if (wide)
        hipLaunchKernelGGL(state_prepare4_kernel, dim3((chunks + kPrepareChunksPerBlock - 1) / kPrepareChunksPerBlock),
                           dim3(kBlock), 0, s, reinterpret_cast<const vf4*>(live), reinterpret_cast<const vf4*>(canonical),
                           reinterpret_cast<vf4*>(state_a), reinterpret_cast<vf4*>(state_b), n, chunks, make_grid(grid),
                           grid->dims, sums_interior, sums_boundary, prepare_masks(scratch, chunks),
                           prepare_opposite(scratch, chunks), prepare_nonempty(scratch, chunks));
    else
        hipLaunchKernelGGL(state_prepare_kernel, dim3(chunks), dim3(kBlock), 0, s, live, canonical,
                           reinterpret_cast<vf4*>(state_a), reinterpret_cast<vf4*>(state_b), n, make_grid(grid), grid->dims,
                           sums_interior, sums_boundary, prepare_masks(scratch, chunks), prepare_opposite(scratch, chunks),
                           prepare_nonempty(scratch, chunks));
    const unsigned tiles = prepare_scan_tiles(chunks) > 0u ? prepare_scan_tiles(chunks) : 1u;
    hipLaunchKernelGGL(band_tile_totals_kernel, dim3(tiles, 3), dim3(1024), 0, s, scratch, chunks, chunks + 1,
                       (const int*)prepare_opposite(scratch, chunks), prepare_tile_totals(scratch, chunks), tiles);
    hipLaunchKernelGGL(band_scan_tiles_kernel, dim3(tiles, 3), dim3(1024), 0, s, scratch, chunks, chunks + 1,
                       (const int*)prepare_tile_totals(scratch, chunks), tiles, (long long*)counts_out, zero_fifth ? 1 : 0);
    return launch_status();
}

static long long pack_group_min_voxels() {
    const char* text = std::getenv("LSF_SPARSE_MIN_VOXELS");
    if (!text || !*text) return 1ll << 21;
    char* end = nullptr;
    const long long value = std::strtoll(text, &end, 10);
    return end && *end == 0 && value >= 0 ? value : 1ll << 21;
}

extern "C" int lsf_state_pack_needed(const float* live, float* state_a, float* state_b, const lsf_grid* grid,
                                     int32_t* scratch, int32_t reach, int32_t invert, void* stream) {
    if (int e = check_grid(grid, true)) return e;
    if (!live || (!state_a && !state_b) || !scratch || reach < 1 || reach > 8) return LSF_ERR_BAD_ARGUMENT;
    if (grid->z_begin != 0 || grid->z_end != grid->nz) return LSF_ERR_BAD_ARGUMENT;
    unsigned first, n, chunks;
    band_range(grid, first, n, chunks);
    hipLaunchKernelGGL(state_pack_needed_kernel, dim3(chunks), dim3(kBlock), 0, as_stream(stream), live,
                       reinterpret_cast<vf4*>(state_a), reinterpret_cast<vf4*>(state_b), n, chunks,
                       prepare_needed(scratch, chunks), invert ? 0 : 1, invert ? 0 : (int)reach, (long long)grid->nx,
                       (long long)grid->nx * grid->ny, grid->dims, (const int*)prepare_nonempty(scratch, chunks),
                       (const unsigned long long*)prepare_masks(scratch, chunks),
                       (long long)n >= pack_group_min_voxels() ? 1 : 0);
    return launch_status();
}

extern "C" int lsf_band_list_fill(const float* live, const float* canonical, const lsf_grid* grid, int32_t subset,
                                  const int32_t* scratch, int32_t* list, void* stream) {
    if (int e = check_grid(grid)) return e;
    if (!live || !canonical || !scratch || !list || !band_subset_ok(subset)) return LSF_ERR_BAD_ARGUMENT;
    unsigned first, n, chunks;
    if (!band_range(grid, first, n, chunks)) return 0;
    hipLaunchKernelGGL(band_list_kernel<true>, dim3(chunks), dim3(kBlock), 0, as_stream(stream), live, canonical, first, n,
                       make_grid(grid), grid->dims, subset, const_cast<int32_t*>(scratch), list);
    return launch_status();
}
```

levelsetfusion-python_amd/csrc/lsf_slavcheva_run.hip:

```cpp
#include "lsf_device.h"

#include <cstring>

using namespace lsf;

namespace {

__global__ __launch_bounds__(kBlock) void records_used_words_kernel(const long long* __restrict__ records,
                                                                    const long long* __restrict__ statistics16,
                                                                    long long* __restrict__ out, int n_slots, int tail) {
    const int k = blockIdx.x * kBlock + threadIdx.x;
    if (k < n_slots * 4) out[k] = records[(long long)(k >> 2) * (sizeof(lsf_record_slot) / 8) + (k & 3)];
    else if (tail && k < n_slots * 4 + 16) out[k] = statistics16 ? statistics16[k - n_slots * 4] : 0ll;
}

__global__ __launch_bounds__(kBlock) void records_from_rows_kernel(const RecordRow* __restrict__ rows,
                                                                   unsigned rows_per_iteration,
                                                                   lsf_iteration_record* __restrict__ records) {
    const RecordRow* mine = rows + (size_t)blockIdx.x * rows_per_iteration;
    unsigned long long best = 0ull;
    double sums[3] = {0.0, 0.0, 0.0};
    for (unsigned r = threadIdx.x; r < rows_per_iteration; r += kBlock) {
        const RecordRow row = mine[r];
        best = row.max_packed > best ? row.max_packed : best;
        sums[0] += row.data;
        sums[1] += row.smoothing;
        sums[2] += row.level_set;
    }
    __shared__ unsigned long long s_max[kBlock / kWave];
    __shared__ double s_sum[3][kBlock / kWave];
    const int lane = threadIdx.x & (kWave - 1), wave = threadIdx.x / kWave;
    best = wave_max_u64(best);
#pragma unroll
    for (int j = 0; j < 3; ++j) sums[j] = wave_sum_f64(sums[j]);
    if (lane == 0) {
        s_max[wave] = best;
#pragma unroll
        for (int j = 0; j < 3; ++j) s_sum[j][wave] = sums[j];
    }
    __syncthreads();
    lsf_iteration_record* record = records + blockIdx.x;
    if (threadIdx.x == 0) {
        unsigned long long m = 0ull;
        double t[3] = {0.0, 0.0, 0.0};
        for (int k = 0; k < kBlock / kWave; ++k) {
            m = s_max[k] > m ? s_max[k] : m;
#pragma unroll
            for (int j = 0; j < 3; ++j) t[j] += s_sum[j][k];
        }
        record->slot[0].max_packed = m;
        record->slot[0].data_energy = t[0];
        record->slot[0].smoothing_energy = t[1];
        record->slot[0].level_set_energy = t[2];
    } else if (threadIdx.x < LSF_RECORD_SLOTS) {
        record->slot[threadIdx.x].max_packed = 0ull;
        record->slot[threadIdx.x].data_energy = 0.0;
        record->slot[threadIdx.x].smoothing_energy = 0.0;
        record->slot[threadIdx.x].level_set_energy = 0.0;
    }
}

inline int64_t rows_per_iteration_max(const lsf_grid* g, int32_t n_lists) {
    const unsigned list = state_iteration_rows_max(g), boxes = state_iteration_boxes_rows_max(g);
    return (int64_t)(list > boxes ? list : boxes) + (n_lists > 1 ? (int64_t)list : 0);
}

inline hipEvent_t thread_event() {
    thread_local hipEvent_t events[64] = {};
    int dev = 0;
    if (hipGetDevice(&dev) != hipSuccess || dev < 0 || dev >= 64) return nullptr;
    if (!events[dev] && hipEventCreateWithFlags(&events[dev], hipEventDisableTiming) != hipSuccess) events[dev] = nullptr;
    return events[dev];
}

inline bool run_ok(const lsf_state_run* r) {
    return r && r->live && r->canonical && r->state[0] && r->state[1] && r->state[0] != r->state[1] && r->prepare_scratch &&
           r->totals_device && r->totals_host && r->sparse_reach >= 0 && r->sparse_reach <= 8;
}

inline int finalize_and_gather_words(const float* final_state, const float* canonical, float* live_out, const lsf_grid* g,
                                     const int32_t* const* listed, const int64_t* listed_counts, int n_listed,
                                     int64_t opposite_count, int64_t first_opposite, float lower_threshold,
                                     double* statistics16, double* finalize_scratch, const lsf_iteration_record* guard_records,
                                     int32_t guard_count, float guard_limit, const lsf_iteration_record* records, int n_slots,
                                     int64_t* words_device, hipStream_t s) {
    if (int e = state_finalize_listed_launch(final_state, canonical, live_out, nullptr, g, listed, listed_counts, n_listed,
                                             opposite_count, first_opposite, lower_threshold, statistics16, finalize_scratch,
                                             nullptr, guard_records, guard_count, guard_limit, statistics16 ? records : nullptr,
                                             statistics16 ? n_slots : 0, statistics16 ? words_device : nullptr, s))
        return e;
    if (statistics16) return 0;
    hipLaunchKernelGGL(records_used_words_kernel, dim3((n_slots * 4 + 16 + kBlock - 1) / kBlock), dim3(kBlock), 0, s,
                       reinterpret_cast<const long long*>(records), (const long long*)nullptr,
                       reinterpret_cast<long long*>(words_device), n_slots, 1);
    return launch_status();
}

}

extern "C" int64_t lsf_state_run_rows_elements(const lsf_grid* grid, int32_t iterations, int32_t n_lists) {
    if (check_grid(grid) || iterations < 1 || n_lists < 1 || n_lists > 2) return 0;
    return rows_per_iteration_max(grid, n_lists) * iterations * (int64_t)(sizeof(RecordRow) / sizeof(int64_t));
}

extern "C" int lsf_state_run_begin(const lsf_state_run* run, void* stream) {
    if (!run_ok(run)) return LSF_ERR_BAD_ARGUMENT;
    const lsf_grid* g = &run->grid;
    if (int e = check_grid(g)) return e;
    if (g->z_begin != 0 || g->z_end != g->nz) return LSF_ERR_BAD_ARGUMENT;
    hipStream_t s = as_stream(stream);
    const bool sparse = run->sparse_reach > 0;
    float* b_in_pass = (sparse || run->second_state_late) ? nullptr : run->state[1];
    if (int e = state_prepare_launch(run->live, run->canonical, sparse ? nullptr : run->state[0], b_in_pass, g,
                                     run->prepare_scratch, run->totals_device, !run->box_scratch, stream))
        return e;
    if (run->box_scratch)
        if (int e = lsf_band_boxes_count(g, run->box_all ? LSF_BAND_ALL : LSF_BAND_INTERIOR, run->prepare_scratch, run->box_scratch,
                                         run->totals_device + 4, stream))
            return e;
    if (hipMemcpyAsync(run->totals_host, run->totals_device, 5 * sizeof(int64_t), hipMemcpyDeviceToHost, s) != hipSuccess)
        return (int)hipGetLastError();
    hipEvent_t sizes = thread_event();
    if (!sizes) return (int)hipGetLastError();
    int status = 0;
    if (hipEventRecord(sizes, s) != hipSuccess) status = (int)hipGetLastError();
    if (!status && sparse)
        status = lsf_state_pack_needed(run->live, run->state[0], run->state[1], g, run->prepare_scratch, run->sparse_reach, 0,
                                       stream);
    else if (!status && run->second_state_late)
        status = lsf_state_pack(run->live, nullptr, run->state[1], nullptr, g, stream);
    if (!status && hipEventSynchronize(sizes) != hipSuccess) status = (int)hipGetLastError();
    return status;
}

extern "C" int lsf_state_run_finish(const lsf_state_run* run, const lsf_slavcheva_params* params, int32_t* list_interior,
                                    int32_t* list_boundary, lsf_band_box* boxes, float* box_canonical,
                                    lsf_iteration_record* records, int32_t iterations, const lsf_run_loop* loop,
                                    float* live_out, float lower_threshold, double* statistics16,
                                    double* finalize_scratch, int64_t* words_device, int64_t* words_host,
                                    lsf_state_run_result* result, void* stream) {
    return lsf_state_run_finish_rows(run, params, list_interior, list_boundary, boxes, box_canonical, records, iterations, loop,
                                     live_out, lower_threshold, statistics16, finalize_scratch, words_device, words_host,
                                     result, nullptr, 0, nullptr, stream);
}

extern "C" int lsf_state_run_finish_rows(const lsf_state_run* run, const lsf_slavcheva_params* params, int32_t* list_interior,
                                         int32_t* list_boundary, lsf_band_box* boxes, float* box_canonical,
                                         lsf_iteration_record* records, int32_t iterations, const lsf_run_loop* loop,
                                         float* live_out, float lower_threshold, double* statistics16,
                                         double* finalize_scratch, int64_t* words_device, int64_t* words_host,
                                         lsf_state_run_result* result, int64_t* record_rows, int64_t record_rows_elements,
                                         int32_t* rows_taken, void* stream) {
    if (rows_taken) *rows_taken = 0;
    if (record_rows && (record_rows_elements <= 0 || (reinterpret_cast<uintptr_t>(record_rows) & 31u) != 0))
        return LSF_ERR_BAD_ARGUMENT;
    if (!run_ok(run) || !params || !records || iterations < 1 || !live_out || !words_device || !words_host || !result ||
        (statistics16 && !finalize_scratch) || !result->max_value || !result->argmax ||
        !result->energies3 || !result->executed)
        return LSF_ERR_BAD_ARGUMENT;
    if (loop && (loop->min_iterations < 1 || loop->check_interval < 1 ||
                 (loop->max_iterations > loop->min_iterations ? loop->max_iterations : loop->min_iterations) != iterations))
        return LSF_ERR_BAD_ARGUMENT;
    if (run->box_all && boxes) return LSF_ERR_BAD_ARGUMENT;
    const lsf_grid* g = &run->grid;
    if (int e = check_grid(g)) return e;
    const int64_t n_interior = run->totals_host[0], n_boundary = run->totals_host[1];
    if (n_interior < 0 || n_boundary < 0 || n_interior > 0x7fffffffll || n_boundary > 0x7fffffffll ||
        (n_interior && !list_interior) || (n_boundary && !list_boundary))
        return LSF_ERR_BAD_ARGUMENT;
    const bool fixed = !loop || loop->min_iterations >= iterations;
    RecordRow* const rows = fixed ? reinterpret_cast<RecordRow*>(record_rows) : nullptr;
    const int64_t rows_capacity = rows ? record_rows_elements / (int64_t)(sizeof(RecordRow) / sizeof(int64_t)) : 0;
    if (rows && record_rows_elements <
                    lsf_state_run_rows_elements(g, iterations, (n_interior ? 1 : 0) + ((n_boundary || !n_interior) ? 1 : 0)))
        return LSF_ERR_BAD_ARGUMENT;
    hipStream_t s = as_stream(stream);
    const int32_t* lists[2];
    int64_t counts[2];
    int32_t subsets[2];
    int n_lists = 0;
    if (n_interior) {
        if (int e = lsf_band_list_fill_prepared(g, LSF_BAND_INTERIOR, run->prepare_scratch, list_interior, stream)) return e;
        lists[n_lists] = list_interior; counts[n_lists] = n_interior; subsets[n_lists++] = LSF_BAND_INTERIOR;
    }
    if (n_boundary || !n_lists) {
        if (n_boundary)
            if (int e = lsf_band_list_fill_prepared(g, LSF_BAND_BOUNDARY, run->prepare_scratch, list_boundary, stream)) return e;
        lists[n_lists] = n_boundary ? list_boundary : reinterpret_cast<const int32_t*>(run->prepare_scratch);
        counts[n_lists] = n_boundary; subsets[n_lists++] = LSF_BAND_BOUNDARY;
    }
    const int64_t n_boxes = boxes && run->box_scratch ? run->totals_host[4] : 0;
    if (n_boxes > 0) {
        if (!box_canonical) return LSF_ERR_BAD_ARGUMENT;
        if (int e = lsf_band_boxes_fill(g, LSF_BAND_INTERIOR, run->prepare_scratch, run->box_scratch, boxes, stream)) return e;
        if (int e = lsf_band_boxes_canonical(run->canonical, g, boxes, n_boxes, box_canonical, stream)) return e;
    }
    const bool sparse = run->sparse_reach > 0;
    const int n_slots = iterations * LSF_RECORD_SLOTS;
    unsigned rows_per_iteration = 0u;
    int32_t it = 0, n_exec = fixed ? iterations : 0;
    while (it < iterations) {
        const int32_t batch = fixed ? iterations : (loop->check_interval < iterations - it ? loop->check_interval : iterations - it);
        for (int32_t i = it; i < it + batch; ++i) {
            lsf_gate gate_i{records + (i > 0 ? i - 1 : 0), LSF_GATE_SLAVCHEVA, loop ? loop->lower_threshold : 0.0f,
                            loop ? loop->upper_threshold : 0.0f};
            const lsf_gate* gate = (fixed || i < loop->min_iterations) ? nullptr : &gate_i;
            int64_t row = (int64_t)i * rows_per_iteration;
            for (int k = 0; k < n_lists; ++k) {
                int e;
                unsigned written = 0u;
                const unsigned room = rows ? (unsigned)(rows_capacity - row < 0x7fffffffll ? rows_capacity - row : 0x7fffffffll) : 0u;
                if (n_boxes > 0 && subsets[k] == LSF_BAND_INTERIOR)
                    e = state_iteration_boxes_launch(run->state[i % 2], box_canonical, run->state[(i + 1) % 2], g, params, gate,
                                                     records + i, boxes, n_boxes, rows ? rows + row : nullptr, room, &written,
                                                     stream);
                else
                    e = state_iteration_launch(run->state[i % 2], run->canonical, run->state[(i + 1) % 2], g, params, gate,
                                               records + i, lists[k], counts[k], subsets[k], rows ? rows + row : nullptr, room,
                                               &written, stream);
                if (e) return e;
                row += written;
            }
            if (i == 0) rows_per_iteration = (unsigned)row;
            else if (rows && row != (int64_t)(i + 1) * rows_per_iteration) return LSF_ERR_BAD_ARGUMENT;
        }
        it += batch;
        if (rows) {
            if (rows_per_iteration == 0u) return LSF_ERR_BAD_ARGUMENT;
            hipLaunchKernelGGL(records_from_rows_kernel, dim3((unsigned)iterations), dim3(kBlock), 0, s, rows, rows_per_iteration,
                               records);
            if (int e = launch_status()) return e;
        }
        if (fixed) break;
        const int first_slot = (it - batch) * LSF_RECORD_SLOTS, batch_slots = batch * LSF_RECORD_SLOTS;
        hipLaunchKernelGGL(records_used_words_kernel, dim3((batch_slots * 4 + kBlock - 1) / kBlock), dim3(kBlock), 0, s,
                           reinterpret_cast<const long long*>(records + (it - batch)), nullptr,
                           reinterpret_cast<long long*>(words_device) + (size_t)first_slot * 4, batch_slots, 0);
        if (int e = launch_status()) return e;
        if (hipMemcpyAsync(words_host + (size_t)first_slot * 4, words_device + (size_t)first_slot * 4,
                           (size_t)batch_slots * 4 * sizeof(int64_t), hipMemcpyDeviceToHost, s) != hipSuccess)
            return (int)hipGetLastError();
        if (hipStreamSynchronize(s) != hipSuccess) return (int)hipGetLastError();
        if (int e = lsf_records_decode(words_host, it, LSF_RECORD_SLOTS, 4, result->max_value, result->argmax,
                                       result->energies3, result->executed))
            return e;
        n_exec = 0;
        while (n_exec < it && result->executed[n_exec]) ++n_exec;
        if (n_exec < it) break;
        const float m = result->max_value[n_exec - 1];
        if (n_exec >= loop->min_iterations && !(loop->lower_threshold < m && m < loop->upper_threshold)) break;
    }
    const float* final_state = run->state[n_exec % 2];
    int64_t listed_counts[2] = {0, 0};
    const int32_t* listed[2] = {nullptr, nullptr};
    int n_listed = 0;
    for (int k = 0; k < n_lists; ++k)
        if (counts[k]) { listed[n_listed] = lists[k]; listed_counts[n_listed++] = counts[k]; }
    if (int e = finalize_and_gather_words(final_state, run->canonical, live_out, g, listed, listed_counts, n_listed,
                                          run->totals_host[2], run->totals_host[3], lower_threshold, statistics16,
                                          finalize_scratch, sparse ? records : nullptr, sparse ? iterations : 0,
                                          (float)run->sparse_reach, records, n_slots, words_device, s))
        return e;
    if (hipMemcpyAsync(words_host, words_device, ((size_t)n_slots * 4 + 16) * sizeof(int64_t), hipMemcpyDeviceToHost, s) !=
        hipSuccess)
        return (int)hipGetLastError();
    if (hipStreamSynchronize(s) != hipSuccess) return (int)hipGetLastError();
    if (int e = lsf_records_decode(words_host, iterations, LSF_RECORD_SLOTS, 4, result->max_value, result->argmax,
                                   result->energies3, result->executed))
        return e;
    result->final_state = n_exec % 2;
    result->n_lists = n_lists;
    result->reach_exceeded = 0;
    result->compact_faces = -1;
    if (rows_taken) *rows_taken = rows ? 1 : 0;
    for (int32_t i = 0; i < iterations && sparse; ++i)
        if (result->executed[i] && !(result->max_value[i] < (float)run->sparse_reach)) result->reach_exceeded = 1;
    return 0;
}

extern "C" int lsf_sobolev_run_finish(const lsf_state_run* run, const lsf_slavcheva_params* params, const double* taps_host,
                                      int32_t n_taps, int32_t* list_interior, int32_t* list_boundary, int32_t* list_all,
                                      lsf_band_box* boxes, float* g4_a, float* g4_b, lsf_iteration_record* records,
                                      int32_t iterations, const lsf_run_loop* loop, float* live_out, float lower_threshold,
                                      double* statistics16, double* finalize_scratch, int64_t* words_device,
                                      int64_t* words_host, lsf_state_run_result* result, void* stream) {
    if (!run_ok(run) || !run->box_scratch || !run->box_all || !params || !taps_host || !boxes || !g4_a || !g4_b ||
        g4_a == g4_b || !records || iterations < 1 || !live_out || !words_device || !words_host || !result ||
        (statistics16 && !finalize_scratch) || !result->max_value || !result->argmax || !result->energies3 ||
        !result->executed)
        return LSF_ERR_BAD_ARGUMENT;
    if (loop && (loop->min_iterations < 1 || loop->check_interval < 1 ||
                 (loop->max_iterations > loop->min_iterations ? loop->max_iterations : loop->min_iterations) != iterations))
        return LSF_ERR_BAD_ARGUMENT;
    const lsf_grid* g = &run->grid;
    if (int e = check_grid(g)) return e;
    if (g->dims != 3) return LSF_ERR_BAD_DIMS;
    const int64_t n_interior = run->totals_host[0], n_boundary = run->totals_host[1], n_boxes = run->totals_host[4];
    if (n_interior < 0 || n_boundary < 0 || n_boxes < 0 || n_interior + n_boundary > 0x7fffffffll ||
        (n_interior && !list_interior) || (n_boundary && !list_boundary) || (n_interior && n_boundary && !list_all))
        return LSF_ERR_BAD_ARGUMENT;
    hipStream_t s = as_stream(stream);
    if (n_interior)
        if (int e = lsf_band_list_fill_prepared(g, LSF_BAND_INTERIOR, run->prepare_scratch, list_interior, stream)) return e;
    if (n_boundary)
        if (int e = lsf_band_list_fill_prepared(g, LSF_BAND_BOUNDARY, run->prepare_scratch, list_boundary, stream)) return e;
    const int32_t* all = n_interior ? list_interior : list_boundary;
    const int64_t n_all = n_interior + n_boundary;
    if (n_interior && n_boundary) {
        const int32_t* a[1] = {list_interior};
        const int32_t* b[1] = {list_boundary};
        int32_t* out[1] = {list_all};
        const int64_t na[1] = {n_interior}, nb[1] = {n_boundary};
        if (int e = lsf_merge_sorted_runs(a, na, b, nb, out, 1, stream)) return e;
        all = list_all;
    }
    if (n_boxes > 0)
        if (int e = lsf_band_boxes_fill(g, LSF_BAND_ALL, run->prepare_scratch, run->box_scratch, boxes, stream)) return e;
    const bool sparse = run->sparse_reach > 0;
    const int n_slots = iterations * LSF_RECORD_SLOTS;
    const bool fixed = !loop || loop->min_iterations >= iterations;
    int32_t it = 0, n_exec = fixed ? iterations : 0;
    while (it < iterations) {
        const int32_t batch = fixed ? iterations : (loop->check_interval < iterations - it ? loop->check_interval : iterations - it);
        for (int32_t i = it; i < it + batch; ++i) {
            lsf_gate gate_i{records + (i > 0 ? i - 1 : 0), LSF_GATE_SLAVCHEVA, loop ? loop->lower_threshold : 0.0f,
                            loop ? loop->upper_threshold : 0.0f};
            const lsf_gate* gate = (fixed || i < loop->min_iterations) ? nullptr : &gate_i;
            const float* s_in = run->state[i % 2];
            float* s_out = run->state[(i + 1) % 2];
            if (n_all)
                if (int e = lsf_sobolev_state_gradient_x(s_in, run->canonical, g4_a, g, params, taps_host, n_taps, gate,
                                                         records + i, all, n_all, 1, stream))
                    return e;
            float* g_out = (!fixed || i == iterations - 1) ? g4_b : nullptr;
            if (int e = lsf_sobolev_state_update_boxes(g4_a, s_in, s_out, g_out, g, params, taps_host, n_taps, gate, records + i,
                                                       boxes, n_boxes, stream))
                return e;
        }
        it += batch;
        if (fixed) break;
        const int first_slot = (it - batch) * LSF_RECORD_SLOTS, batch_slots = batch * LSF_RECORD_SLOTS;
        hipLaunchKernelGGL(records_used_words_kernel, dim3((batch_slots * 4 + kBlock - 1) / kBlock), dim3(kBlock), 0, s,
                           reinterpret_cast<const long long*>(records + (it - batch)), nullptr,
                           reinterpret_cast<long long*>(words_device) + (size_t)first_slot * 4, batch_slots, 0);
        if (int e = launch_status()) return e;
        if (hipMemcpyAsync(words_host + (size_t)first_slot * 4, words_device + (size_t)first_slot * 4,
                           (size_t)batch_slots * 4 * sizeof(int64_t), hipMemcpyDeviceToHost, s) != hipSuccess)
            return (int)hipGetLastError();
        if (hipStreamSynchronize(s) != hipSuccess) return (int)hipGetLastError();
        if (int e = lsf_records_decode(words_host, it, LSF_RECORD_SLOTS, 4, result->max_value, result->argmax,
                                       result->energies3, result->executed))
            return e;
        n_exec = 0;
        while (n_exec < it && result->executed[n_exec]) ++n_exec;
        if (n_exec < it) break;
        const float m = result->max_value[n_exec - 1];
        if (n_exec >= loop->min_iterations && !(loop->lower_threshold < m && m < loop->upper_threshold)) break;
    }
    const int32_t* listed[2] = {nullptr, nullptr};
    int64_t listed_counts[2] = {0, 0};
    int n_listed = 0;
    if (n_interior) { listed[n_listed] = list_interior; listed_counts[n_listed++] = n_interior; }
    if (n_boundary) { listed[n_listed] = list_boundary; listed_counts[n_listed++] = n_boundary; }
    if (int e = finalize_and_gather_words(run->state[n_exec % 2], run->canonical, live_out, g, listed, listed_counts, n_listed,
                                          run->totals_host[2], run->totals_host[3], lower_threshold, statistics16,
                                          finalize_scratch, sparse ? records : nullptr, sparse ? iterations : 0,
                                          (float)run->sparse_reach, records, n_slots, words_device, s))
        return e;
    if (hipMemcpyAsync(words_host, words_device, ((size_t)n_slots * 4 + 16) * sizeof(int64_t), hipMemcpyDeviceToHost, s) !=
        hipSuccess)
        return (int)hipGetLastError();
    if (hipStreamSynchronize(s) != hipSuccess) return (int)hipGetLastError();
    if (int e = lsf_records_decode(words_host, iterations, LSF_RECORD_SLOTS, 4, result->max_value, result->argmax,
                                   result->energies3, result->executed))
        return e;
    result->final_state = n_exec % 2;
    result->n_lists = n_listed;
    result->reach_exceeded = 0;
    result->compact_faces = -1;
    for (int32_t i = 0; i < iterations && sparse; ++i)
        if (result->executed[i] && !(result->max_value[i] < (float)run->sparse_reach)) result->reach_exceeded = 1;
    return 0;
}
```

levelsetfusion-python_amd/engine_options.py:

```python
import os
import types

SLAVCHEVA_DEFAULTS = dict(
    use_band_list=True,
    library_run=True,
    record_rows=True,
    box_walk=None,
    sobolev_boxes=True,
    sparse_reach=None,
    sparse_min_voxels=None,
    box_walk_min_band_bytes=100 * 1000 * 1000,
    box_walk_min_voxels=1 << 25,
)

HIERARCHICAL_DEFAULTS = dict(
    use_graphs=True,
    graph_max_voxels=1 << 21,
    fused_filter=True,
    fused_filter_min_voxels=1 << 23,
    defer_maximum=True,
    blocked_levels=True,
)


def apply(engine, defaults, options):
    options = dict(options or {})
    unknown = sorted(set(options) - set(defaults))
    if unknown:
        raise TypeError("unknown engine option(s) %s (known: %s)" % (", ".join(unknown), ", ".join(sorted(defaults))))
    for name, value in defaults.items():
        setattr(engine, name, options.get(name, value))
    if "sparse_reach" in defaults:
        if engine.sparse_reach is None:
            engine.sparse_reach = int(os.environ.get("LSF_SPARSE_REACH", "2"))
        if engine.sparse_min_voxels is None:
            engine.sparse_min_voxels = int(os.environ.get("LSF_SPARSE_MIN_VOXELS", str(1 << 21)))


def new_call_report():
    return types.SimpleNamespace(sparse_states=False, box_walk=False, sobolev_boxes=False, library_run=False,
                                 blocked_levels=0, record_rows=False, route=None)
```

levelsetfusion-python_amd/engine_run.py:

```python
import ctypes

import numpy as np
import torch

from . import _lib, device as dev
from .engine_common import _Fast, _Lazy
from .engine_outcome import _RunLog, _RunOutcome, recompute_gradient


class _SparseStateExceeded(Exception):
    """a call whose ping-pong states were initialised near the band only (dev.StatePrepare(sparse_reach=...)) met a warp
    update that can read beyond that; nothing of the caller's has been modified (SlavchevaEngine.optimize repeats the
    call on fully initialised states and keeps doing so for this optimizer)"""


class _RunCall:

    def __init__(self, engine, live, canonical, grid, finalize, sparse, base, totals_name, n_totals, restore=False):
        live_out = finalize[0]
        self.engine, self.canonical, self.grid = engine, canonical, grid
        device = self.device = live.device
        n = self.n = dev.n_voxels(grid)
        whole = self.whole = dev.full_range(grid)
        engine.last_call.sparse_states = sparse
        engine.last_call.library_run = True
        usable = (live_out is not None and live_out.is_cuda and live_out.dtype == torch.float32
                  and live_out.is_contiguous() and tuple(live_out.shape) == tuple(live.shape))
        target = self.target = live_out if usable else torch.empty_like(live)
        if target is not live:
            target.copy_(live)
        elif usable and restore:
            engine._slab_restore = (live_out, live_out.clone())
        states = self.states = [torch.empty(tuple(live.shape) + (4,), dtype=torch.float32, device=device)
                                for _ in range(2)]
        self.scratch = torch.empty(int(_lib.lib.lsf_state_prepare_scratch_elements(ctypes.byref(whole))),
                                   dtype=torch.int32, device=device)
        self.totals = torch.empty(n_totals, dtype=torch.int64, device=device)
        self.totals_host = dev.pinned_scratch(totals_name, n_totals, torch.int64)
        base.live, base.canonical = dev._ptr(live, n, "live"), dev._ptr(canonical, n, "canonical")
        base.state[0], base.state[1] = states[0].data_ptr(), states[1].data_ptr()
        base.prepare_scratch, base.totals_device, base.totals_host = self.scratch.data_ptr(), self.totals.data_ptr(), \
            self.totals_host.data_ptr()
        base.grid = whole
        base.sparse_reach = engine.sparse_reach if sparse else 0
        base.second_state_late = int(not sparse and n <= dev.StatePrepare.SPLIT_MAX_VOXELS)

    def results(self, lists, n_interior, n_boundary, iterations, device_words, host_name, host_words):
        self.lists = lists
        records = self.records = dev.new_records(iterations, self.device)
        self.words = torch.empty(device_words, dtype=torch.int64, device=self.device)
        self.words_host = dev.pinned_scratch(host_name, host_words, torch.int64)
        self.max_value, self.argmax = np.empty(iterations, np.float32), np.empty(iterations, np.int64)
        self.energies, self.executed = np.empty((iterations, 3), np.float64), np.empty(iterations, np.bool_)
        self.result = _lib.StateRunResult(self.max_value.ctypes.data, self.argmax.ctypes.data, self.energies.ctypes.data,
                                          self.executed.ctypes.data)
        bands = self.bands = []
        if n_interior:
            bands.append(dev.BandList(lists[:n_interior], n_interior, _lib.BAND_INTERIOR))
        if n_boundary or not bands:
            bands.append(dev.BandList(lists[n_interior:] if n_boundary else lists[:1], n_boundary, _lib.BAND_BOUNDARY))
        fast = self.fast = _Fast(self.grid, records, bands=bands)
        self.outcome = _RunOutcome(self.grid, self.canonical, None, self.target, bands, None)
        self.weights = tuple(self.engine.weights)
        return fast

    def leave(self, gradient_grid, gradient=None, n_exec=None):
        e = self.engine
        if n_exec is None:
            n_exec = len(self.executed) if self.executed.all() else int(self.executed.sum())
        e._fast = self.fast
        e.iteration_count = n_exec
        e.log = _RunLog(self.max_value[:n_exec], self.argmax[:n_exec], self.energies[:n_exec], self.weights)
        if gradient is None:
            params, state_in, canonical, bands = e.params, self.states[(n_exec - 1) % 2], self.canonical, self.bands
            gradient = _Lazy(lambda: recompute_gradient(params, state_in, canonical, gradient_grid, bands))
        e._gradient_state = gradient
        self.outcome.state = self.states[n_exec % 2]
        return self.outcome


class RunMixin:

    def _optimize_run(self, live, canonical, grid, finalize, sobolev=False):
        live_out, lower_threshold, statistics = finalize
        iterations = max(self.min_iterations, self.max_iterations)
        loop = None
        if self.min_iterations < iterations:
            loop = _lib.RunLoop(self.min_iterations, self.max_iterations, self.lo, self.hi, self.check_interval, 0)
        run = _lib.StateRun()
        c = _RunCall(self, live, canonical, grid, finalize, self._sparse_states(grid), run, "run totals", 5)
        device, n, whole = c.device, c.n, c.whole
        count_boxes = sobolev or (dev.boxes_ok(whole) and (self.box_walk is True or
                                                           (self.box_walk is None and n >= self.box_walk_min_voxels)))
        run.box_all = int(sobolev)
        box_scratch = None
        if count_boxes:
            box_scratch = torch.empty(int(_lib.lib.lsf_band_boxes_scratch_elements(ctypes.byref(whole))),
                                      dtype=torch.int32, device=device)
            run.box_scratch = box_scratch.data_ptr()
        stream = dev.stream_ptr()
        _lib.check(_lib.lib.lsf_state_run_begin(ctypes.byref(run), stream), "lsf_state_run_begin")
        n_interior, n_boundary, opposite, first_opposite, n_boxes = c.totals_host.tolist()
        lists = torch.empty(max(n_interior + n_boundary, 1), dtype=torch.int32, device=device)
        boxes = box_canonical = None
        if sobolev:
            boxes = torch.empty((max(n_boxes, 1), 2), dtype=torch.int64, device=device)
            list_all = torch.empty(max(n_interior + n_boundary, 1), dtype=torch.int32, device=device) \
                if n_interior and n_boundary else None
            g4 = self._sobolev_gradient_buffers(live, whole, lists, n_interior + n_boundary)
            taps = np.ascontiguousarray(np.asarray(self.sobolev_kernel, dtype=np.float64))
            self.last_call.sobolev_boxes = True
        elif n_boxes and (self.box_walk is True or 32 * n_interior > self.box_walk_min_band_bytes):
            boxes = torch.empty((n_boxes, 2), dtype=torch.int64, device=device)
            box_canonical = torch.empty(n_boxes * dev.BOX_EDGE ** 3, dtype=torch.float32, device=device)
        self.last_call.box_walk = boxes is not None and not sobolev
        record_rows = None
        if loop is None and not sobolev and self.record_rows:
            n_launches = int(n_interior > 0) + int(n_boundary > 0 or n_interior == 0)
            record_rows = torch.empty(int(_lib.lib.lsf_state_run_rows_elements(ctypes.byref(whole), iterations, n_launches)),
                                      dtype=torch.int64, device=device)
        n_words = iterations * _lib.RECORD_SLOTS * dev.USED_SLOT_WORDS
        f = c.results(lists, n_interior, n_boundary, iterations, n_words + 16, "run records", n_words + 16)
        records, words, words_host, result = c.records, c.words, c.words_host, c.result
        stats = stats_scratch = None
        if statistics:
            stats = torch.empty(16, dtype=torch.float64, device=device)
            stats_scratch = torch.empty(2 * int(_lib.lib.lsf_state_finalize_scratch_elements(ctypes.byref(whole))),
                                        dtype=torch.float64, device=device)
        none = ctypes.c_void_p(0)
        p_lists = lists.data_ptr()
        f.boxes = (boxes, box_canonical)
        if sobolev:
            f.keep = (g4, list_all, taps)
            self._sobolev_band = f
            _lib.check(_lib.lib.lsf_sobolev_run_finish(
                ctypes.byref(run), ctypes.byref(self.params), taps.ctypes.data_as(ctypes.POINTER(ctypes.c_double)),
                int(taps.size), ctypes.c_void_p(p_lists), ctypes.c_void_p(p_lists + 4 * n_interior),
                ctypes.c_void_p(list_all.data_ptr() if list_all is not None else 0), ctypes.c_void_p(boxes.data_ptr()),
                ctypes.c_void_p(g4[0].data_ptr()), ctypes.c_void_p(g4[1].data_ptr()), ctypes.c_void_p(records.data_ptr()),
                iterations, ctypes.byref(loop) if loop is not None else None, dev._ptr(c.target, n, "live_out"),
                float(lower_threshold), ctypes.c_void_p(stats.data_ptr()) if statistics else none,
                ctypes.c_void_p(stats_scratch.data_ptr()) if statistics else none, ctypes.c_void_p(words.data_ptr()),
                ctypes.c_void_p(words_host.data_ptr()), ctypes.byref(result), stream), "lsf_sobolev_run_finish")
        else:
            self._run_finish(run, p_lists, n_interior, boxes, box_canonical, records, iterations, loop, c.target, n,
                             lower_threshold, stats, stats_scratch, statistics, words, words_host, result, stream, record_rows)
        if result.reach_exceeded:
            raise _SparseStateExceeded()
        outcome = c.leave(grid, _Lazy(lambda: g4[1][..., :grid.dims].movedim(-1, 0).contiguous()) if sobolev else None)
        if statistics:
            outcome._raw = words_host[n_words:].numpy().view(np.float64).copy()
        return outcome

    def _sobolev_gradient_buffers(self, live, whole, lists, n_listed):
        key = (tuple(live.shape), live.device)
        cache = self._g4_cache
        if cache is not None and cache[0] == key:
            _, g4, old_lists, old_n = cache
            for t, bricks in ((g4[0], 1), (g4[1], 0)):
                _lib.check(_lib.lib.lsf_zero_listed4(ctypes.c_void_p(t.data_ptr()), ctypes.byref(whole),
                                                     ctypes.c_void_p(old_lists.data_ptr()), old_n, bricks, dev.stream_ptr()),
                           "lsf_zero_listed4")
        else:
            self._g4_cache = None
            g4 = [torch.zeros(tuple(live.shape) + (4,), dtype=torch.float32, device=live.device) for _ in range(2)]
        self._g4_cache = (key, g4, lists, int(n_listed))
        return g4

    def _run_finish(self, run, p_lists, n_interior, boxes, box_canonical, records, iterations, loop, target, n,
                    lower_threshold, stats, stats_scratch, statistics, words, words_host, result, stream, record_rows=None):
        none = ctypes.c_void_p(0)
        rows_taken = ctypes.c_int32(0)
        _lib.check(_lib.lib.lsf_state_run_finish_rows(
            ctypes.byref(run), ctypes.byref(self.params), ctypes.c_void_p(p_lists),
            ctypes.c_void_p(p_lists + 4 * n_interior), ctypes.c_void_p(boxes.data_ptr() if boxes is not None else 0),
            ctypes.c_void_p(box_canonical.data_ptr() if boxes is not None else 0),
            ctypes.c_void_p(records.data_ptr()), iterations, ctypes.byref(loop) if loop is not None else None,
            dev._ptr(target, n, "live_out"), float(lower_threshold),
            ctypes.c_void_p(stats.data_ptr()) if statistics else none,
            ctypes.c_void_p(stats_scratch.data_ptr()) if statistics else none, ctypes.c_void_p(words.data_ptr()),
            ctypes.c_void_p(words_host.data_ptr()), ctypes.byref(result),
            ctypes.c_void_p(record_rows.data_ptr()) if record_rows is not None else none,
            record_rows.numel() if record_rows is not None else 0, ctypes.byref(rows_taken), stream),
            "lsf_state_run_finish_rows")
        self.last_call.record_rows = bool(rows_taken.value)
```

levelsetfusion-python_amd/engine_slavcheva.py:

```python
import collections
import ctypes

import numpy as np
import torch

from . import _lib, device as dev, engine_options
from .engine_common import _Counted, _Fast, _Lazy
from .engine_focus import FocusMixin
from .engine_outcome import _StateIteration, recompute_gradient
from .engine_run import RunMixin, _SparseStateExceeded
from .engine_slab import SlabMixin, _HaloTooNarrow
from .engine_sobolev import _PlanarIteration, _SobolevStatePlan

ROUTES = ("library_run", "library_sobolev_run", "library_slab_run", "launches")

_LaunchPlan = collections.namedtuple("_LaunchPlan", "planar_sobolev sob_state fused_prepare slab_groups sparse warp_fill "
                                                    "sobolev_boxes")


class _FusedIteration(_StateIteration):

    def __init__(self, engine, launcher, limit, psi=None, complete=None):
        self.engine, self.f, self.limit, self.psi, self._complete = engine, launcher, limit, psi, complete

    def enqueue(self, i):
        e, f = self.engine, self.f
        if e._slab():
            return e._enqueue_slab_state_iteration(i, self.states, self.limit)
        s_in, s_out = f.p_state[i % 2], f.p_state[(i + 1) % 2]
        gate_ref = None if i < e.min_iterations else f.gate_ref(i - 1)
        run = _lib.lib.lsf_slavcheva_state_iteration
        for band in f.bands:
            status = run(s_in, f.p_canon, s_out, f.grid_ref, f.params_ref, gate_ref, f.record_ptrs[i],
                         band.pointer, band.count, band.subset, f.stream)
            if status:
                _lib.check(status, "lsf_slavcheva_state_iteration")
        run = _lib.lib.lsf_cumulative_warp_compose
        for band in f.bands if self.psi is not None else ():
            if band.indices is not None and band.count == 0:
                continue
            status = run(f.p_state[(i + 1) % 2], f.p_psi[i % 2], f.p_psi[(i + 1) % 2], f.grid_ref, gate_ref, band.pointer,
                         band.count, f.stream)
            if status:
                _lib.check(status, "lsf_cumulative_warp_compose")

    def _recompute(self, state_in, complete=None):
        params, canonical, grid = self.engine.params, self.canonical, self.grid
        return _Lazy(lambda: recompute_gradient(params, state_in, canonical, grid, complete=complete))

    def after(self, i):
        warp_planar = self.inputs(i + 1)[1]
        source = self.engine._gradient_state = self._recompute(self.states[i % 2])
        return warp_planar, source.get()

    def gradient_source(self, n_exec):
        return self._recompute(self.states[(n_exec - 1) % 2], self._complete)

    def cumulative_source(self, n_exec):
        psi, grid = self.psi[n_exec % 2], self.grid

        def interleaved():
            out = torch.empty(tuple(psi.shape[:-1]) + (grid.dims,), dtype=torch.float32, device=psi.device)
            dev.state_unpack(psi, grid, warp_interleaved_out=out)
            return out
        return _Lazy(interleaved)


class SlavchevaEngine(RunMixin, SlabMixin, FocusMixin):

    def __init__(self, direct, level_set_term_enabled, sobolev_smoothing_enabled, data_term_method,
                 smoothing_term_method, gradient_descent_rate, data_term_weight, smoothing_term_weight,
                 isomorphic_enforcement_factor, level_set_term_weight, lower_threshold, upper_threshold,
                 max_iterations, min_iterations, sobolev_kernel, compute_energies=True, check_interval=32,
                 comm=None, options=None, cumulative_warp=False):
        self.direct = bool(direct)
        self.sobolev = bool(sobolev_smoothing_enabled)
        self.sobolev_kernel = sobolev_kernel
        if self.sobolev and sobolev_kernel is None:
            raise ValueError("sobolev_smoothing_enabled requires a sobolev_kernel")
        self.cumulative_warp = bool(cumulative_warp)
        if self.cumulative_warp and self.sobolev:
            raise ValueError("cumulative_warp does not combine with sobolev_smoothing_enabled: the planar and float4 "
                             "Sobolev launch plans do not compose the warp")
        if self.cumulative_warp and comm is not None and comm.active:
            raise ValueError("cumulative_warp does not combine with an active comm: slab runs would need a halo of the "
                             "cumulative warp")
        lam = float(isomorphic_enforcement_factor)
        smoothing = smoothing_term_method if self.direct else _lib.SMOOTHING_TIKHONOV
        data = data_term_method if self.direct else _lib.DATA_BASIC
        level_set = bool(level_set_term_enabled) and self.direct
        energy = _lib.ENERGY_NONE if not compute_energies else \
            (_lib.ENERGY_DIRECT if self.direct else _lib.ENERGY_VECTORIZED)
        self.params = _lib.SlavchevaParams(lam, float(gradient_descent_rate), float(data_term_weight),
                                           float(smoothing_term_weight), float(level_set_term_weight), lam,
                                           float(np.float32(-2.0 * (1.0 + lam))), int(smoothing), int(data),
                                           int(level_set), int(energy), int(self.direct), 0)
        self.weights = (float(data_term_weight), float(smoothing_term_weight), float(level_set_term_weight))
        self.lo, self.hi = float(lower_threshold), float(upper_threshold)
        self.max_iterations, self.min_iterations = int(max_iterations), int(min_iterations)
        self.check_interval = max(1, int(check_interval))
        self.comm = comm
        engine_options.apply(self, engine_options.SLAVCHEVA_DEFAULTS, options)
        self.sparse_disabled = False
        self.iteration_hook = None
        self._declare_call_state()

    def _declare_call_state(self):
        self.last_call = engine_options.new_call_report()
        self.iteration_count = 0
        self.log = None
        self._fast = self._gradient_state = self._cumulative_state = self._sobolev_band = None
        self._g4_cache, self._cut_chunk_cache = None, (None, None)
        self._exchange_every_iteration = False
        self._slab_restore = self._pending_halos = None
        self._comm_stream = self._events = self._plan_stream = self._no_face = None
        self._focus_flat = None

    def _grid(self, live):
        if self.comm is not None and self.comm.active:
            L = self.comm.layout
            if L.axis == 1:
                if live.dim() != 3 or live.shape[1] != L.n_local:
                    raise ValueError("y-slab runs need a 3-D local field with %d rows, got %r"
                                     % (L.n_local, tuple(live.shape)))
                g = dev.make_grid(live.shape)
                g.y_global_offset, g.ny_global = L.global_offset, L.n_global
                g.energy_y_begin, g.energy_y_end = L.begin, L.end
                return g
            if live.dim() != 3 or live.shape[0] != L.nz_local:
                raise ValueError("slab runs need a 3-D local field with %d slices, got %r"
                                 % (L.nz_local, tuple(live.shape)))
            return dev.make_grid(live.shape, L.z_begin, L.z_end, L.z_global_offset)
        return dev.make_grid(live.shape)

    def _slab(self):
        return self.comm is not None and self.comm.active

    def _gate_for(self, records, i):
        return None if i < self.min_iterations else dev.make_gate(records, i - 1, _lib.GATE_SLAVCHEVA, self.lo,
                                                                  self.hi)

    def _sparse_states(self, grid, watched=False):
        if self._slab() and not self._slab_groups():
            return False
        return (self.sparse_reach > 0 and dev.n_voxels(grid) >= self.sparse_min_voxels and not watched
                and not self.sparse_disabled)

    def _slab_groups(self):
        return (self._slab() and self.min_iterations >= max(self.max_iterations, self.min_iterations)
                and not self._exchange_every_iteration and self.comm.layout.halo >= max(self.sparse_reach, 2))

    def _route(self, grid, finalize, watched):
        slab = self._slab()
        run_ok = (self.library_run and finalize is not None and not self.sobolev and self.use_band_list
                  and not watched and self.min_iterations > 0 and dev.buffer_addressing_ok(grid)
                  and not self.cumulative_warp)
        if (self.library_run and finalize is not None and self.sobolev and self.sobolev_boxes and self.use_band_list
                and not watched and self.min_iterations > 0 and not slab and grid.dims == 3
                and dev.boxes_ok(grid) and dev.n_voxels(grid) < (1 << 27) and dev.buffer_addressing_ok(grid)
                and len(self.sobolev_kernel) in dev.LISTED_TAP_COUNTS):
            return "library_sobolev_run"
        if run_ok and not slab:
            return "library_run"
        if run_ok and slab and not finalize[2] and self.min_iterations >= self.max_iterations and self._slab_run_ok(grid):
            return "library_slab_run"
        return "launches"

    def _launch_plan(self, grid, finalize, watched):
        slab = self._slab()
        sob_state = (self.sobolev and self.use_band_list and not slab and dev.buffer_addressing_ok(grid)
                     and len(self.sobolev_kernel) in dev.LISTED_TAP_COUNTS)
        planar_sobolev = self.sobolev and not sob_state
        fused_prepare = not planar_sobolev and self.use_band_list and dev.buffer_addressing_ok(grid)
        fill_first = dev.n_voxels(grid) <= (1 << 24)
        fill = fused_prepare and finalize is not None and not slab
        warp_fill = ("before" if fill_first else "behind") if fill else None
        boxes = (sob_state and fused_prepare and not slab and self.sobolev_boxes and _SobolevStatePlan.fuses_x(grid)
                 and dev.boxes_ok(grid) and dev.n_voxels(grid) < (1 << 27)
                 and len(self.sobolev_kernel) in dev.LISTED_TAP_COUNTS)
        return _LaunchPlan(planar_sobolev, sob_state, fused_prepare, fused_prepare and self._slab_groups(),
                           fused_prepare and self._sparse_states(grid, watched), warp_fill, boxes)

    def optimize(self, live, canonical, finalize=None):
        if not self._slab():
            try:
                return self._optimize(live, canonical, finalize)
            except _SparseStateExceeded:
                self.sparse_disabled = True
                torch.cuda.synchronize()
                return self._optimize(live, canonical, finalize)
        self._slab_restore = None
        try:
            outcome = self._optimize(live, canonical, finalize)
            self._slab_restore = None
            return outcome
        except _HaloTooNarrow as exc:
            torch.cuda.synchronize()
            if self._slab_restore is not None:
                self._slab_restore[0].copy_(self._slab_restore[1])
                self._slab_restore = None
            return self._optimize_widened(live, canonical, exc.max_update)

    def _optimize(self, live, canonical, finalize=None):
        if live.shape != canonical.shape:
            raise ValueError("live and canonical fields must have the same shape")
        self._gradient_state = None
        self._cumulative_state = None
        self._fast = None
        self.last_call = engine_options.new_call_report()
        grid = self._grid(live)
        watched = self.iteration_hook is not None or self.focus_voxels is not None
        if self.focus_voxels is not None:
            self._focus_begin(live, canonical)
        route = self.last_call.route = self._route(grid, finalize, watched)
        if route in ("library_run", "library_sobolev_run"):
            return self._optimize_run(live, canonical, grid, finalize, sobolev=route == "library_sobolev_run")
        if route == "library_slab_run":
            return self._optimize_slab_run(live, canonical, grid, finalize)
        if self._slab():
            need = 1 if not self.sobolev else max(1, len(self.sobolev_kernel) // 2)
            if self.comm.layout.halo < need:
                raise ValueError("slab halo of %d slices is too narrow: this configuration needs >= %d"
                                 % (self.comm.layout.halo, need))
        plan = self._launch_plan(grid, finalize, watched)
        limit = 0 if self.min_iterations == 0 else max(self.max_iterations, self.min_iterations)
        iteration = self._set_up(live, canonical, grid, finalize, plan, limit)
        n_exec, dec = self._run_batches(iteration, plan, finalize, limit, watched)
        return self._leave_behind(iteration, n_exec, dec, limit)

    def _slab_cut_chunks(self, live, grid):
        if not (self._slab() and self.comm.layout.axis == 0 and (grid.ny * grid.nx) % dev.StatePrepare.CHUNK == 0):
            return None
        zs = self._slab_cut_slices(grid)
        key = (tuple(zs), grid.ny * grid.nx, live.device)
        if self._cut_chunk_cache[0] != key:
            per_slice = grid.ny * grid.nx // dev.StatePrepare.CHUNK
            self._cut_chunk_cache = (key, torch.tensor([z * per_slice for z in zs], dtype=torch.int64,
                                                       device=live.device))
        return self._cut_chunk_cache[1]

    def _set_up(self, live, canonical, grid, finalize, plan, limit):
        slab, dims = self._slab(), grid.dims
        prepared = warp_zeroed = None
        if plan.fused_prepare:
            cut_chunks = self._slab_cut_chunks(live, grid)
            if plan.warp_fill == "before":
                warp_zeroed = torch.zeros(tuple(live.shape) + (dims,), dtype=torch.float32, device=live.device)
            self.last_call.sparse_states = plan.sparse
            prepared = dev.StatePrepare(live, canonical, dev.full_range(grid), cut_chunks,
                                        sparse_reach=self.sparse_reach if plan.sparse else 0)
            if plan.warp_fill == "behind":
                warp_zeroed = torch.zeros(tuple(live.shape) + (dims,), dtype=torch.float32, device=live.device)
        live_at_entry = None
        if slab and finalize is not None and finalize[0] is not None and not plan.planar_sobolev \
                and self.min_iterations >= max(self.max_iterations, self.min_iterations):
            live_at_entry = finalize[0].clone()
        records = dev.new_records(max(self.max_iterations, self.min_iterations, 1), live.device)
        if plan.planar_sobolev:
            iteration = _PlanarIteration(self, live, canonical, grid, records, limit)
            self._sobolev_band = iteration.band
            return iteration
        listed = None
        states = prepared.states if plan.fused_prepare else dev.state_pack(live, None, grid, copies=2)
        n = dev.n_voxels(grid)
        f = _Fast(grid, records, gate=(_lib.GATE_SLAVCHEVA, self.lo, self.hi))
# ... 106 lines not shown
```

Measured before the change: 552.1 billion.

## Add single-call state run with bounded list fill and mapped host writes

Result: slower. 541.3 billion (-2.0%).

```diff
diff --git a/include/lsf_hip.h b/include/lsf_hip.h
--- a/include/lsf_hip.h
+++ b/include/lsf_hip.h
@@ -259,6 +259,12 @@
                               int64_t *words_host, lsf_state_run_result *result, int64_t *record_rows,
                               int64_t record_rows_elements, int32_t *rows_taken, void *stream);
 int64_t lsf_state_run_rows_elements(const lsf_grid *grid, int32_t iterations, int32_t n_lists);
+#define LSF_RUN_NEEDS_CAPACITY 0x40000000
+int lsf_state_run_call(const lsf_state_run *run, const lsf_slavcheva_params *params, int32_t *lists, int64_t list_capacity,
+                       lsf_iteration_record *records, int32_t iterations, const lsf_run_loop *loop, float *live_out,
+                       float lower_threshold, double *statistics16, double *finalize_scratch, int64_t *words_device,
+                       int64_t *words_host, lsf_state_run_result *result, int64_t *record_rows,
+                       int64_t record_rows_elements, int32_t *rows_taken, void *stream);
 
 int lsf_sobolev_run_finish(const lsf_state_run *run, const lsf_slavcheva_params *params, const double *taps_host,
                            int32_t n_taps, int32_t *list_interior, int32_t *list_boundary, int32_t *list_all,
diff --git a/levelsetfusion-python_amd/_lib.py b/levelsetfusion-python_amd/_lib.py
--- a/levelsetfusion-python_amd/_lib.py
+++ b/levelsetfusion-python_amd/_lib.py
@@ -9,10 +9,12 @@
 
 MAX_KERNEL_TAPS = 31
 ABI_VERSION = 4
-HEADER_ABI_HASH = "7b9c31a7c45631ef"
+HEADER_ABI_HASH = "b172d94b7d6f20ea"
 
 ERRORS = {-1: "LSF_ERR_BAD_ARGUMENT", -2: "LSF_ERR_BAD_DIMS", -3: "LSF_ERR_KERNEL_TOO_LONG",
           -4: "LSF_ERR_RCCL_UNAVAILABLE", -5: "LSF_ERR_RCCL_FAILED", -6: "LSF_ERR_NOT_RESIDENT"}
+
+RUN_NEEDS_CAPACITY = 0x40000000
 
 SMOOTHING_TIKHONOV, SMOOTHING_KILLING = 0, 1
 DATA_BASIC, DATA_THRESHOLDED_FDM = 0, 2
@@ -440,6 +442,9 @@
                                                  _vp, _f32, _vp, _vp, _vp, _vp, _P(StateRunResult), _vp, ctypes.c_int64,
                                                  _P(ctypes.c_int32), _vp]),
     "lsf_state_run_rows_elements": (ctypes.c_int64, [_P(Grid), _i32, _i32]),
+    "lsf_state_run_call": (ctypes.c_int, [_P(StateRun), _P(SlavchevaParams), _vp, ctypes.c_int64, _vp, _i32, _P(RunLoop), _vp,
+                                          _f32, _vp, _vp, _vp, _vp, _P(StateRunResult), _vp, ctypes.c_int64,
+                                          _P(ctypes.c_int32), _vp]),
     "lsf_state_run_finish": (ctypes.c_int, [_P(StateRun), _P(SlavchevaParams), _vp, _vp, _vp, _vp, _vp, _i32, _P(RunLoop), _vp,
                                             _f32, _vp, _vp, _vp, _vp, _P(StateRunResult), _vp]),
     "lsf_sobolev_run_finish": (ctypes.c_int, [_P(StateRun), _P(SlavchevaParams), _P(ctypes.c_double), _i32, _vp, _vp, _vp, _vp,
diff --git a/levelsetfusion-python_amd/csrc/lsf_device.h b/levelsetfusion-python_amd/csrc/lsf_device.h
--- a/levelsetfusion-python_amd/csrc/lsf_device.h
+++ b/levelsetfusion-python_amd/csrc/lsf_device.h
@@ -611,7 +611,9 @@
                                  const lsf_band_box* boxes, int64_t box_count, RecordRow* rows, unsigned rows_capacity,
                                  unsigned* rows_written, void* stream);
 int state_prepare_launch(const float* live, const float* canonical, float* state_a, float* state_b, const lsf_grid* grid,
-                         int32_t* scratch, int64_t* counts_out, bool zero_fifth, void* stream);
+                         int32_t* scratch, int64_t* counts_out, bool zero_fifth, int64_t* counts_mirror, void* stream);
+int band_lists_fill_bounded(const lsf_grid* grid, const int32_t* scratch, int32_t* lists, int64_t capacity,
+                            const int64_t* interior_total, void* stream);
 unsigned state_iteration_rows_max(const lsf_grid* grid);
 unsigned state_iteration_boxes_rows_max(const lsf_grid* grid);
 int state_finalize_listed_launch(const float* state, const float* canonical, float* live_out, float* warp_interleaved_out,
diff --git a/levelsetfusion-python_amd/csrc/lsf_slavcheva.hip b/levelsetfusion-python_amd/csrc/lsf_slavcheva.hip
--- a/levelsetfusion-python_amd/csrc/lsf_slavcheva.hip
+++ b/levelsetfusion-python_amd/csrc/lsf_slavcheva.hip
@@ -406,11 +406,13 @@
 
 __global__ __launch_bounds__(1024) void band_scan_tiles_kernel(int* __restrict__ sums_base, unsigned n, unsigned stride,
                                                                const int* __restrict__ tile_out, unsigned tiles,
-                                                               long long* __restrict__ totals, int zero_fifth) {
+                                                               long long* __restrict__ totals,
+                                                               long long* __restrict__ totals_mirror, int zero_fifth) {
     const unsigned tile = blockIdx.x, a = blockIdx.y, t = threadIdx.x, lane = t & (kWave - 1), wave = t / kWave;
     if (a == 2u) {
         if (tile == 0u && t == 0u) {
             if (zero_fifth) totals[4] = 0;
+            if (zero_fifth && totals_mirror) totals_mirror[4] = 0;
             long long sum = 0;
             int first = 0x7fffffff;
             for (unsigned k = 0; k < tiles; ++k) {
@@ -419,6 +421,10 @@
             }
             totals[2] = sum;
             totals[3] = first == 0x7fffffff ? -1 : first;
+            if (totals_mirror) {
+                totals_mirror[2] = sum;
+                totals_mirror[3] = first == 0x7fffffff ? -1 : first;
+            }
         }
         return;
     }
@@ -452,7 +458,10 @@
         if (i + k < n) sums[i + k] = run;
         run += v[k];
     }
-    if (tile == tiles - 1u && t == 0u) totals[a] = (long long)carry + whole;
+    if (tile == tiles - 1u && t == 0u) {
+        totals[a] = (long long)carry + whole;
+        if (totals_mirror) totals_mirror[a] = (long long)carry + whole;
+    }
 }
 
 typedef float vf4 __attribute__((ext_vector_type(4)));
@@ -716,21 +725,25 @@
 }
 
 __global__ __launch_bounds__(kBlock) void band_fill_from_masks_kernel(const unsigned long long* __restrict__ masks,
-                                                                      const int* __restrict__ block_sums, int which,
-                                                                      int* __restrict__ list, unsigned chunks) {
+                                                                      const int* __restrict__ sums_base, unsigned stride,
+                                                                      int which, int* __restrict__ list, unsigned chunks,
+                                                                      const long long* __restrict__ boundary_base,
+                                                                      unsigned capacity) {
     const int lane = threadIdx.x % kWave;
     const unsigned chunk = blockIdx.x * (kBlock / kWave) + threadIdx.x / kWave;
     if (chunk >= chunks) return;
+    which += (int)blockIdx.y;
     const unsigned long long mine = lane < 16 ? masks[((size_t)chunk * 16 + lane) * 2 + which] : 0ull;
     if (__ballot(mine != 0ull) == 0ull) return;
-    int at = block_sums[chunk];
+    int at = sums_base[(size_t)which * stride + chunk];
+    if (which == 1 && boundary_base) at += (int)*boundary_base;
 #pragma unroll
     for (int w = 0; w < 16; ++w) {
         const unsigned lo = (unsigned)__shfl((int)(unsigned)mine, w, kWave);
         const unsigned hi = (unsigned)__shfl((int)(unsigned)(mine >> 32), w, kWave);
         const unsigned long long m = ((unsigned long long)hi << 32) | lo;
-        if ((m >> lane) & 1ull)
-            list[at + __popcll(m & ((1ull << lane) - 1ull))] = (int)(chunk * kBandChunk + w * kWave + lane);
+        const unsigned to = (unsigned)(at + __popcll(m & ((1ull << lane) - 1ull)));
+        if (((m >> lane) & 1ull) && to < capacity) list[to] = (int)(chunk * kBandChunk + w * kWave + lane);
         at += __popcll(m);
     }
 }
@@ -895,8 +908,22 @@
     if (!band_range(grid, first, n, chunks)) return 0;
     const int which = subset == LSF_BAND_INTERIOR ? 0 : 1;
     hipLaunchKernelGGL(band_fill_from_masks_kernel, dim3((chunks + kBlock / kWave - 1) / (kBlock / kWave)), dim3(kBlock),
-                       0, as_stream(stream), prepare_masks(const_cast<int32_t*>(scratch), chunks),
-                       scratch + which * (size_t)(chunks + 1), which, list, chunks);
+                       0, as_stream(stream), prepare_masks(const_cast<int32_t*>(scratch), chunks), scratch, chunks + 1u, which,
+                       list, chunks, (const long long*)nullptr, 0xffffffffu);
+    return launch_status();
+}
+
+int lsf::band_lists_fill_bounded(const lsf_grid* grid, const int32_t* scratch, int32_t* lists, int64_t capacity,
+                                 const int64_t* interior_total, void* stream) {
+    if (int e = check_grid(grid, true)) return e;
+    if (!scratch || !lists || !interior_total || capacity < 1 || capacity > 0x7fffffffll || grid->z_begin != 0 ||
+        grid->z_end != grid->nz)
+        return LSF_ERR_BAD_ARGUMENT;
+    unsigned first, n, chunks;
+    if (!band_range(grid, first, n, chunks)) return 0;
+    hipLaunchKernelGGL(band_fill_from_masks_kernel, dim3((chunks + kBlock / kWave - 1) / (kBlock / kWave), 2), dim3(kBlock),
+                       0, as_stream(stream), prepare_masks(const_cast<int32_t*>(scratch), chunks), scratch, chunks + 1u, 0,
+                       lists, chunks, reinterpret_cast<const long long*>(interior_total), (unsigned)capacity);
     return launch_status();
 }
 
@@ -998,11 +1025,11 @@
 
 extern "C" int lsf_state_prepare(const float* live, const float* canonical, float* state_a, float* state_b,
                                  const lsf_grid* grid, int32_t* scratch, int64_t* counts_out, void* stream) {
-    return state_prepare_launch(live, canonical, state_a, state_b, grid, scratch, counts_out, false, stream);
+    return state_prepare_launch(live, canonical, state_a, state_b, grid, scratch, counts_out, false, nullptr, stream);
 }
 
 int lsf::state_prepare_launch(const float* live, const float* canonical, float* state_a, float* state_b, const lsf_grid* grid,
-                              int32_t* scratch, int64_t* counts_out, bool zero_fifth, void* stream) {
+                              int32_t* scratch, int64_t* counts_out, bool zero_fifth, int64_t* counts_mirror, void* stream) {
     if (int e = check_grid(grid, true)) return e;
     if (!live || !canonical || (!state_a && state_b) || !scratch || !counts_out) return LSF_ERR_BAD_ARGUMENT;
     if (grid->z_begin != 0 || grid->z_end != grid->nz) return LSF_ERR_BAD_ARGUMENT;
@@ -1027,7 +1054,8 @@
     hipLaunchKernelGGL(band_tile_totals_kernel, dim3(tiles, 3), dim3(1024), 0, s, scratch, chunks, chunks + 1,
                        (const int*)prepare_opposite(scratch, chunks), prepare_tile_totals(scratch, chunks), tiles);
     hipLaunchKernelGGL(band_scan_tiles_kernel, dim3(tiles, 3), dim3(1024), 0, s, scratch, chunks, chunks + 1,
-                       (const int*)prepare_tile_totals(scratch, chunks), tiles, (long long*)counts_out, zero_fifth ? 1 : 0);
+                       (const int*)prepare_tile_totals(scratch, chunks), tiles, (long long*)counts_out,
+                       (long long*)counts_mirror, zero_fifth ? 1 : 0);
     return launch_status();
 }
 
diff --git a/levelsetfusion-python_amd/csrc/lsf_slavcheva_run.hip b/levelsetfusion-python_amd/csrc/lsf_slavcheva_run.hip
--- a/levelsetfusion-python_amd/csrc/lsf_slavcheva_run.hip
+++ b/levelsetfusion-python_amd/csrc/lsf_slavcheva_run.hip
@@ -73,6 +73,26 @@
     return events[dev];
 }
 
+inline void* host_as_device(void* host) {
+    constexpr int kKept = 8;
+    thread_local void* seen[kKept] = {};
+    thread_local void* view[kKept] = {};
+    thread_local int seen_device[kKept] = {};
+    thread_local unsigned next = 0u;
+    int dev = 0;
+    if (!host || hipGetDevice(&dev) != hipSuccess) return nullptr;
+    for (int k = 0; k < kKept; ++k)
+        if (seen[k] == host && seen_device[k] == dev) return view[k];
+    void* d = nullptr;
+    if (hipHostGetDevicePointer(&d, host, 0) != hipSuccess) {
+        (void)hipGetLastError();
+        d = nullptr;
+    }
+    const unsigned at = next++ % kKept;
+    seen[at] = host; seen_device[at] = dev; view[at] = d;
+    return d;
+}
+
 inline bool run_ok(const lsf_state_run* r) {
     return r && r->live && r->canonical && r->state[0] && r->state[1] && r->state[0] != r->state[1] && r->prepare_scratch &&
            r->totals_device && r->totals_host && r->sparse_reach >= 0 && r->sparse_reach <= 8;
@@ -83,17 +103,24 @@
                                      int64_t opposite_count, int64_t first_opposite, float lower_threshold,
                                      double* statistics16, double* finalize_scratch, const lsf_iteration_record* guard_records,
                                      int32_t guard_count, float guard_limit, const lsf_iteration_record* records, int n_slots,
-                                     int64_t* words_device, hipStream_t s) {
+                                     int64_t* words_device, int64_t* words_host, hipStream_t s) {
+    int64_t* const direct = static_cast<int64_t*>(host_as_device(words_host));
+    int64_t* const words_out = direct ? direct : words_device;
     if (int e = state_finalize_listed_launch(final_state, canonical, live_out, nullptr, g, listed, listed_counts, n_listed,
                                              opposite_count, first_opposite, lower_threshold, statistics16, finalize_scratch,
                                              nullptr, guard_records, guard_count, guard_limit, statistics16 ? records : nullptr,
-                                             statistics16 ? n_slots : 0, statistics16 ? words_device : nullptr, s))
-        return e;
-    if (statistics16) return 0;
-    hipLaunchKernelGGL(records_used_words_kernel, dim3((n_slots * 4 + 16 + kBlock - 1) / kBlock), dim3(kBlock), 0, s,
-                       reinterpret_cast<const long long*>(records), (const long long*)nullptr,
-                       reinterpret_cast<long long*>(words_device), n_slots, 1);
-    return launch_status();
+                                             statistics16 ? n_slots : 0, statistics16 ? words_out : nullptr, s))
+        return e;
+    if (!statistics16) {
+        hipLaunchKernelGGL(records_used_words_kernel, dim3((n_slots * 4 + 16 + kBlock - 1) / kBlock), dim3(kBlock), 0, s,
+                           reinterpret_cast<const long long*>(records), (const long long*)nullptr,
+                           reinterpret_cast<long long*>(words_out), n_slots, 1);
+        if (int e = launch_status()) return e;
+    }
+    if (!direct && hipMemcpyAsync(words_host, words_device, ((size_t)n_slots * 4 + 16) * sizeof(int64_t),
+                                  hipMemcpyDeviceToHost, s) != hipSuccess)
+        return (int)hipGetLastError();
+    return 0;
 }
 
 }
@@ -103,7 +130,9 @@
     return rows_per_iteration_max(grid, n_lists) * iterations * (int64_t)(sizeof(RecordRow) / sizeof(int64_t));
 }
 
-extern "C" int lsf_state_run_begin(const lsf_state_run* run, void* stream) {
+namespace {
+
+int run_begin(const lsf_state_run* run, int32_t* lists, int64_t list_capacity, void* stream) {
     if (!run_ok(run)) return LSF_ERR_BAD_ARGUMENT;
     const lsf_grid* g = &run->grid;
     if (int e = check_grid(g)) return e;
@@ -111,14 +140,16 @@
     hipStream_t s = as_stream(stream);
     const bool sparse = run->sparse_reach > 0;
     float* b_in_pass = (sparse || run->second_state_late) ? nullptr : run->state[1];
+    int64_t* const totals_direct = run->box_scratch ? nullptr : static_cast<int64_t*>(host_as_device(run->totals_host));
     if (int e = state_prepare_launch(run->live, run->canonical, sparse ? nullptr : run->state[0], b_in_pass, g,
-                                     run->prepare_scratch, run->totals_device, !run->box_scratch, stream))
+                                     run->prepare_scratch, run->totals_device, !run->box_scratch, totals_direct, stream))
         return e;
     if (run->box_scratch)
         if (int e = lsf_band_boxes_count(g, run->box_all ? LSF_BAND_ALL : LSF_BAND_INTERIOR, run->prepare_scratch, run->box_scratch,
                                          run->totals_device + 4, stream))
             return e;
-    if (hipMemcpyAsync(run->totals_host, run->totals_device, 5 * sizeof(int64_t), hipMemcpyDeviceToHost, s) != hipSuccess)
+    if (!totals_direct &&
+        hipMemcpyAsync(run->totals_host, run->totals_device, 5 * sizeof(int64_t), hipMemcpyDeviceToHost, s) != hipSuccess)
         return (int)hipGetLastError();
     hipEvent_t sizes = thread_event();
     if (!sizes) return (int)hipGetLastError();
@@ -129,29 +160,17 @@
                                        stream);
     else if (!status && run->second_state_late)
         status = lsf_state_pack(run->live, nullptr, run->state[1], nullptr, g, stream);
+    if (!status && lists)
+        status = band_lists_fill_bounded(g, run->prepare_scratch, lists, list_capacity, run->totals_device, stream);
     if (!status && hipEventSynchronize(sizes) != hipSuccess) status = (int)hipGetLastError();
     return status;
 }
 
-extern "C" int lsf_state_run_finish(const lsf_state_run* run, const lsf_slavcheva_params* params, int32_t* list_interior,
-                                    int32_t* list_boundary, lsf_band_box* boxes, float* box_canonical,
-                                    lsf_iteration_record* records, int32_t iterations, const lsf_run_loop* loop,
-                                    float* live_out, float lower_threshold, double* statistics16,
-                                    double* finalize_scratch, int64_t* words_device, int64_t* words_host,
-                                    lsf_state_run_result* result, void* stream) {
-    return lsf_state_run_finish_rows(run, params, list_interior, list_boundary, boxes, box_canonical, records, iterations, loop,
-                                     live_out, lower_threshold, statistics16, finalize_scratch, words_device, words_host,
-                                     result, nullptr, 0, nullptr, stream);
-}
-
-extern "C" int lsf_state_run_finish_rows(const lsf_state_run* run, const lsf_slavcheva_params* params, int32_t* list_interior,
-                                         int32_t* list_boundary, lsf_band_box* boxes, float* box_canonical,
-                                         lsf_iteration_record* records, int32_t iterations, const lsf_run_loop* loop,
-                                         float* live_out, float lower_threshold, double* statistics16,
-                                         double* finalize_scratch, int64_t* words_device, int64_t* words_host,
-                                         lsf_state_run_result* result, int64_t* record_rows, int64_t record_rows_elements,
-                                         int32_t* rows_taken, void* stream) {
-    if (rows_taken) *rows_taken = 0;
+int finish_arguments(const lsf_state_run* run, const lsf_slavcheva_params* params, const lsf_band_box* boxes,
+                     const lsf_iteration_record* records, int32_t iterations, const lsf_run_loop* loop, const float* live_out,
+                     const double* statistics16, const double* finalize_scratch, const int64_t* words_device,
+                     const int64_t* words_host, const lsf_state_run_result* result, const int64_t* record_rows,
+                     int64_t record_rows_elements) {
     if (record_rows && (record_rows_elements <= 0 || (reinterpret_cast<uintptr_t>(record_rows) & 31u) != 0))
         return LSF_ERR_BAD_ARGUMENT;
     if (!run_ok(run) || !params || !records || iterations < 1 || !live_out || !words_device || !words_host || !result ||
@@ -162,8 +181,19 @@
                  (loop->max_iterations > loop->min_iterations ? loop->max_iterations : loop->min_iterations) != iterations))
         return LSF_ERR_BAD_ARGUMENT;
     if (run->box_all && boxes) return LSF_ERR_BAD_ARGUMENT;
+    return check_grid(&run->grid);
+}
+
+int run_finish(const lsf_state_run* run, const lsf_slavcheva_params* params, int32_t* list_interior, int32_t* list_boundary,
+               bool lists_filled, lsf_band_box* boxes, float* box_canonical, lsf_iteration_record* records,
+               int32_t iterations, const lsf_run_loop* loop, float* live_out, float lower_threshold, double* statistics16,
+               double* finalize_scratch, int64_t* words_device, int64_t* words_host, lsf_state_run_result* result,
+               int64_t* record_rows, int64_t record_rows_elements, int32_t* rows_taken, void* stream) {
+    if (rows_taken) *rows_taken = 0;
+    if (int e = finish_arguments(run, params, boxes, records, iterations, loop, live_out, statistics16, finalize_scratch,
+                                 words_device, words_host, result, record_rows, record_rows_elements))
+        return e;
     const lsf_grid* g = &run->grid;
-    if (int e = check_grid(g)) return e;
     const int64_t n_interior = run->totals_host[0], n_boundary = run->totals_host[1];
     if (n_interior < 0 || n_boundary < 0 || n_interior > 0x7fffffffll || n_boundary > 0x7fffffffll ||
         (n_interior && !list_interior) || (n_boundary && !list_boundary))
@@ -180,11 +210,12 @@
     int32_t subsets[2];
     int n_lists = 0;
     if (n_interior) {
-        if (int e = lsf_band_list_fill_prepared(g, LSF_BAND_INTERIOR, run->prepare_scratch, list_interior, stream)) return e;
+        if (!lists_filled)
+            if (int e = lsf_band_list_fill_prepared(g, LSF_BAND_INTERIOR, run->prepare_scratch, list_interior, stream)) return e;
         lists[n_lists] = list_interior; counts[n_lists] = n_interior; subsets[n_lists++] = LSF_BAND_INTERIOR;
     }
     if (n_boundary || !n_lists) {
-        if (n_boundary)
+        if (n_boundary && !lists_filled)
             if (int e = lsf_band_list_fill_prepared(g, LSF_BAND_BOUNDARY, run->prepare_scratch, list_boundary, stream)) return e;
         lists[n_lists] = n_boundary ? list_boundary : reinterpret_cast<const int32_t*>(run->prepare_scratch);
         counts[n_lists] = n_boundary; subsets[n_lists++] = LSF_BAND_BOUNDARY;
@@ -259,11 +290,8 @@
     if (int e = finalize_and_gather_words(final_state, run->canonical, live_out, g, listed, listed_counts, n_listed,
                                           run->totals_host[2], run->totals_host[3], lower_threshold, statistics16,
                                           finalize_scratch, sparse ? records : nullptr, sparse ? iterations : 0,
-                                          (float)run->sparse_reach, records, n_slots, words_device, s))
-        return e;
-    if (hipMemcpyAsync(words_host, words_device, ((size_t)n_slots * 4 + 16) * sizeof(int64_t), hipMemcpyDeviceToHost, s) !=
-        hipSuccess)
-        return (int)hipGetLastError();
+                                          (float)run->sparse_reach, records, n_slots, words_device, words_host, s))
+        return e;
     if (hipStreamSynchronize(s) != hipSuccess) return (int)hipGetLastError();
     if (int e = lsf_records_decode(words_host, iterations, LSF_RECORD_SLOTS, 4, result->max_value, result->argmax,
                                    result->energies3, result->executed))
@@ -276,6 +304,57 @@
     for (int32_t i = 0; i < iterations && sparse; ++i)
         if (result->executed[i] && !(result->max_value[i] < (float)run->sparse_reach)) result->reach_exceeded = 1;
     return 0;
+}
+
+}
+
+extern "C" int lsf_state_run_begin(const lsf_state_run* run, void* stream) { return run_begin(run, nullptr, 0, stream); }
+
+extern "C" int lsf_state_run_call(const lsf_state_run* run, const lsf_slavcheva_params* params, int32_t* lists,
+                                  int64_t list_capacity, lsf_iteration_record* records, int32_t iterations,
+                                  const lsf_run_loop* loop, float* live_out, float lower_threshold, double* statistics16,
+                                  double* finalize_scratch, int64_t* words_device, int64_t* words_host,
+                                  lsf_state_run_result* result, int64_t* record_rows, int64_t record_rows_elements,
+                                  int32_t* rows_taken, void* stream) {
+    if (rows_taken) *rows_taken = 0;
+    if (int e = finish_arguments(run, params, nullptr, records, iterations, loop, live_out, statistics16, finalize_scratch,
+                                 words_device, words_host, result, record_rows, record_rows_elements))
+        return e;
+    if (run->box_scratch || run->box_all || !lists || list_capacity < 1 || list_capacity > 0x7fffffffll)
+        return LSF_ERR_BAD_ARGUMENT;
+    const bool fixed = !loop || loop->min_iterations >= iterations;
+    if (fixed && record_rows && record_rows_elements < lsf_state_run_rows_elements(&run->grid, iterations, 2))
+        return LSF_ERR_BAD_ARGUMENT;
+    if (int e = run_begin(run, lists, list_capacity, stream)) return e;
+    const int64_t n_interior = run->totals_host[0], n_boundary = run->totals_host[1];
+    if (n_interior < 0 || n_boundary < 0) return LSF_ERR_BAD_ARGUMENT;
+    if (n_interior + n_boundary > list_capacity) return LSF_RUN_NEEDS_CAPACITY;
+    return run_finish(run, params, lists, lists + n_interior, true, nullptr, nullptr, records, iterations, loop, live_out,
+                      lower_threshold, statistics16, finalize_scratch, words_device, words_host, result, record_rows,
+                      record_rows_elements, rows_taken, stream);
+}
+
+extern "C" int lsf_state_run_finish(const lsf_state_run* run, const lsf_slavcheva_params* params, int32_t* list_interior,
+                                    int32_t* list_boundary, lsf_band_box* boxes, float* box_canonical,
+                                    lsf_iteration_record* records, int32_t iterations, const lsf_run_loop* loop,
+                                    float* live_out, float lower_threshold, double* statistics16,
+                                    double* finalize_scratch, int64_t* words_device, int64_t* words_host,
+                                    lsf_state_run_result* result, void* stream) {
+    return lsf_state_run_finish_rows(run, params, list_interior, list_boundary, boxes, box_canonical, records, iterations, loop,
+                                     live_out, lower_threshold, statistics16, finalize_scratch, words_device, words_host,
+                                     result, nullptr, 0, nullptr, stream);
+}
+
+extern "C" int lsf_state_run_finish_rows(const lsf_state_run* run, const lsf_slavcheva_params* params, int32_t* list_interior,
+                                         int32_t* list_boundary, lsf_band_box* boxes, float* box_canonical,
+                                         lsf_iteration_record* records, int32_t iterations, const lsf_run_loop* loop,
+                                         float* live_out, float lower_threshold, double* statistics16,
+                                         double* finalize_scratch, int64_t* words_device, int64_t* words_host,
+                                         lsf_state_run_result* result, int64_t* record_rows, int64_t record_rows_elements,
+                                         int32_t* rows_taken, void* stream) {
+    return run_finish(run, params, list_interior, list_boundary, false, boxes, box_canonical, records, iterations, loop,
+                      live_out, lower_threshold, statistics16, finalize_scratch, words_device, words_host, result, record_rows,
+                      record_rows_elements, rows_taken, stream);
 }
 
 extern "C" int lsf_sobolev_run_finish(const lsf_state_run* run, const lsf_slavcheva_params* params, const double* taps_host,
@@ -365,11 +444,8 @@
     if (int e = finalize_and_gather_words(run->state[n_exec % 2], run->canonical, live_out, g, listed, listed_counts, n_listed,
                                           run->totals_host[2], run->totals_host[3], lower_threshold, statistics16,
                                           finalize_scratch, sparse ? records : nullptr, sparse ? iterations : 0,
-                                          (float)run->sparse_reach, records, n_slots, words_device, s))
-        return e;
-    if (hipMemcpyAsync(words_host, words_device, ((size_t)n_slots * 4 + 16) * sizeof(int64_t), hipMemcpyDeviceToHost, s) !=
-        hipSuccess)
-        return (int)hipGetLastError();
+                                          (float)run->sparse_reach, records, n_slots, words_device, words_host, s))
+        return e;
     if (hipStreamSynchronize(s) != hipSuccess) return (int)hipGetLastError();
     if (int e = lsf_records_decode(words_host, iterations, LSF_RECORD_SLOTS, 4, result->max_value, result->argmax,
                                    result->energies3, result->executed))
diff --git a/levelsetfusion-python_amd/engine_options.py b/levelsetfusion-python_amd/engine_options.py
--- a/levelsetfusion-python_amd/engine_options.py
+++ b/levelsetfusion-python_amd/engine_options.py
@@ -1,10 +1,16 @@
 import os
 import types
+
+
+class _CallReport(types.SimpleNamespace):
+    __slots__ = ("foreign_calls", "capacity_fallback")
 
 SLAVCHEVA_DEFAULTS = dict(
     use_band_list=True,
     library_run=True,
     record_rows=True,
+    single_call=True,
+    single_call_capacity=None,
     box_walk=None,
     sobolev_boxes=True,
     sparse_reach=None,
@@ -38,5 +44,7 @@
 
 
 def new_call_report():
-    return types.SimpleNamespace(sparse_states=False, box_walk=False, sobolev_boxes=False, library_run=False,
-                                 blocked_levels=0, record_rows=False, route=None)
+    report = _CallReport(sparse_states=False, box_walk=False, sobolev_boxes=False, library_run=False, blocked_levels=0,
+                         record_rows=False, route=None)
+    report.foreign_calls, report.capacity_fallback = 0, False
+    return report
diff --git a/levelsetfusion-python_amd/engine_run.py b/levelsetfusion-python_amd/engine_run.py
--- a/levelsetfusion-python_amd/engine_run.py
+++ b/levelsetfusion-python_amd/engine_run.py
@@ -44,25 +44,40 @@
         base.grid = whole
         base.sparse_reach = engine.sparse_reach if sparse else 0
         base.second_state_late = int(not sparse and n <= dev.StatePrepare.SPLIT_MAX_VOXELS)
+        self.bands = None
 
     def results(self, lists, n_interior, n_boundary, iterations, device_words, host_name, host_words):
-        self.lists = lists
-        records = self.records = dev.new_records(iterations, self.device)
-        self.words = torch.empty(device_words, dtype=torch.int64, device=self.device)
+        self.buffers(iterations, device_words, host_name, host_words)
+        return self.band_lists(lists, n_interior, n_boundary)
+
+    def buffers(self, iterations, device_words, host_name, host_words, zero_records=True):
+        self.records = dev.new_records(iterations, self.device) if zero_records else \
+            torch.empty((iterations, dev.RECORD_WORDS), dtype=torch.int64, device=self.device)
+        self.words = device_words if isinstance(device_words, torch.Tensor) else \
+            torch.empty(device_words, dtype=torch.int64, device=self.device)
         self.words_host = dev.pinned_scratch(host_name, host_words, torch.int64)
         self.max_value, self.argmax = np.empty(iterations, np.float32), np.empty(iterations, np.int64)
         self.energies, self.executed = np.empty((iterations, 3), np.float64), np.empty(iterations, np.bool_)
         self.result = _lib.StateRunResult(self.max_value.ctypes.data, self.argmax.ctypes.data, self.energies.ctypes.data,
                                           self.executed.ctypes.data)
-        bands = self.bands = []
+        self.weights = tuple(self.engine.weights)
+
+    def outcome_objects(self):
+        self.bands = []
+        self.fast = _Fast(self.grid, self.records, bands=self.bands)
+        self.outcome = _RunOutcome(self.grid, self.canonical, None, self.target, self.bands, None)
+
+    def band_lists(self, lists, n_interior, n_boundary):
+        self.lists = lists
+        if self.bands is None:
+            self.outcome_objects()
+        bands = self.bands
         if n_interior:
             bands.append(dev.BandList(lists[:n_interior], n_interior, _lib.BAND_INTERIOR))
         if n_boundary or not bands:
-            bands.append(dev.BandList(lists[n_interior:] if n_boundary else lists[:1], n_boundary, _lib.BAND_BOUNDARY))
-        fast = self.fast = _Fast(self.grid, records, bands=bands)
-        self.outcome = _RunOutcome(self.grid, self.canonical, None, self.target, bands, None)
-        self.weights = tuple(self.engine.weights)
-        return fast
+            bands.append(dev.BandList(lists[n_interior:n_interior + n_boundary] if n_boundary else lists[:1], n_boundary,
+                                      _lib.BAND_BOUNDARY))
+        return self.fast
 
     def leave(self, gradient_grid, gradient=None, n_exec=None):
         e = self.engine
@@ -99,9 +114,43 @@
                                       dtype=torch.int32, device=device)
             run.box_scratch = box_scratch.data_ptr()
         stream = dev.stream_ptr()
-        _lib.check(_lib.lib.lsf_state_run_begin(ctypes.byref(run), stream), "lsf_state_run_begin")
+        n_words = iterations * _lib.RECORD_SLOTS * dev.USED_SLOT_WORDS
+        rows = loop is None and not sobolev and self.record_rows
+        key = (tuple(live.shape), device)
+        capacity = None
+        if self.single_call and not count_boxes:
+            capacity = self.single_call_capacity if self.single_call_capacity is not None else self._list_capacity.get(key)
+        status, lists, record_rows = None, None, None
+        if capacity is not None:
+            lists = self._new_lists(max(int(capacity), 1), device)
+            scratch_key = (key, iterations, bool(rows), bool(statistics))
+            if self._run_scratch[0] != scratch_key:
+                self._run_scratch = (None, None)
+                kept_rows = torch.empty(int(_lib.lib.lsf_state_run_rows_elements(ctypes.byref(whole), iterations, 2)),
+                                        dtype=torch.int64, device=device) if rows else None
+                self._run_scratch = (scratch_key, (kept_rows, torch.empty(n_words + 16, dtype=torch.int64, device=device))
+                                     + self._statistics_buffers(statistics, whole, device))
+            record_rows, kept_words, stats, stats_scratch = self._run_scratch[1]
+            c.buffers(iterations, kept_words, "run records", n_words + 16, zero_records=not rows)
+            c.outcome_objects()
+            status = self._run_call(run, lists, c.records, iterations, loop, c.target, n, lower_threshold, stats,
+                                    stats_scratch, c.words, c.words_host, c.result, stream, record_rows)
+            self.last_call.capacity_fallback = status == _lib.RUN_NEEDS_CAPACITY
+        else:
+            _lib.check(_lib.lib.lsf_state_run_begin(ctypes.byref(run), stream), "lsf_state_run_begin")
         n_interior, n_boundary, opposite, first_opposite, n_boxes = c.totals_host.tolist()
-        lists = torch.empty(max(n_interior + n_boundary, 1), dtype=torch.int32, device=device)
+        next_capacity = max(n_interior + n_boundary + (n_interior + n_boundary) // 8, 1)
+        self.last_call.foreign_calls = 1 if status == 0 else 2
+        if status == 0:
+            c.band_lists(lists, n_interior, n_boundary)
+            if c.result.reach_exceeded:
+                raise _SparseStateExceeded()
+            self._list_capacity[key] = next_capacity
+            outcome = c.leave(grid)
+            if statistics:
+                outcome._raw = c.words_host[n_words:].numpy().view(np.float64).copy()
+            return outcome
+        lists = self._new_lists(max(n_interior + n_boundary, 1), device)
         boxes = box_canonical = None
         if sobolev:
             boxes = torch.empty((max(n_boxes, 1), 2), dtype=torch.int64, device=device)
@@ -114,19 +163,15 @@
             boxes = torch.empty((n_boxes, 2), dtype=torch.int64, device=device)
             box_canonical = torch.empty(n_boxes * dev.BOX_EDGE ** 3, dtype=torch.float32, device=device)
         self.last_call.box_walk = boxes is not None and not sobolev
-        record_rows = None
-        if loop is None and not sobolev and self.record_rows:
+        if rows and record_rows is None:
             n_launches = int(n_interior > 0) + int(n_boundary > 0 or n_interior == 0)
             record_rows = torch.empty(int(_lib.lib.lsf_state_run_rows_elements(ctypes.byref(whole), iterations, n_launches)),
                                       dtype=torch.int64, device=device)
-        n_words = iterations * _lib.RECORD_SLOTS * dev.USED_SLOT_WORDS
-        f = c.results(lists, n_interior, n_boundary, iterations, n_words + 16, "run records", n_words + 16)
+        if status is None:
+            c.buffers(iterations, n_words + 16, "run records", n_words + 16)
+            stats, stats_scratch = self._statistics_buffers(statistics, whole, device)
+        f = c.band_lists(lists, n_interior, n_boundary)
         records, words, words_host, result = c.records, c.words, c.words_host, c.result
-        stats = stats_scratch = None
-        if statistics:
-            stats = torch.empty(16, dtype=torch.float64, device=device)
-            stats_scratch = torch.empty(2 * int(_lib.lib.lsf_state_finalize_scratch_elements(ctypes.byref(whole))),
-                                        dtype=torch.float64, device=device)
         none = ctypes.c_void_p(0)
         p_lists = lists.data_ptr()
         f.boxes = (boxes, box_canonical)
@@ -147,6 +192,8 @@
                              lower_threshold, stats, stats_scratch, statistics, words, words_host, result, stream, record_rows)
         if result.reach_exceeded:
             raise _SparseStateExceeded()
+        if not count_boxes:
+            self._list_capacity[key] = next_capacity
         outcome = c.leave(grid, _Lazy(lambda: g4[1][..., :grid.dims].movedim(-1, 0).contiguous()) if sobolev else None)
         if statistics:
             outcome._raw = words_host[n_words:].numpy().view(np.float64).copy()
@@ -166,6 +213,35 @@
             g4 = [torch.zeros(tuple(live.shape) + (4,), dtype=torch.float32, device=live.device) for _ in range(2)]
         self._g4_cache = (key, g4, lists, int(n_listed))
         return g4
+
+    def _new_lists(self, entries, device):
+        return torch.empty(entries, dtype=torch.int32, device=device)
+
+    @staticmethod
+    def _statistics_buffers(statistics, whole, device):
+        if not statistics:
+            return None, None
+        return (torch.empty(16, dtype=torch.float64, device=device),
+                torch.empty(2 * int(_lib.lib.lsf_state_finalize_scratch_elements(ctypes.byref(whole))),
+                            dtype=torch.float64, device=device))
+
+    def _run_call(self, run, lists, records, iterations, loop, target, n, lower_threshold, stats, stats_scratch, words,
+                  words_host, result, stream, record_rows):
+        none = ctypes.c_void_p(0)
+        rows_taken = ctypes.c_int32(0)
+        status = _lib.lib.lsf_state_run_call(
+            ctypes.byref(run), ctypes.byref(self.params), ctypes.c_void_p(lists.data_ptr()), lists.numel(),
+            ctypes.c_void_p(records.data_ptr()), iterations, ctypes.byref(loop) if loop is not None else None,
+            dev._ptr(target, n, "live_out"), float(lower_threshold),
+            ctypes.c_void_p(stats.data_ptr()) if stats is not None else none,
+            ctypes.c_void_p(stats_scratch.data_ptr()) if stats is not None else none, ctypes.c_void_p(words.data_ptr()),
+            ctypes.c_void_p(words_host.data_ptr()), ctypes.byref(result),
+            ctypes.c_void_p(record_rows.data_ptr()) if record_rows is not None else none,
+            record_rows.numel() if record_rows is not None else 0, ctypes.byref(rows_taken), stream)
+        if status != _lib.RUN_NEEDS_CAPACITY:
+            _lib.check(status, "lsf_state_run_call")
+        self.last_call.record_rows = bool(rows_taken.value)
+        return status
 
     def _run_finish(self, run, p_lists, n_interior, boxes, box_canonical, records, iterations, loop, target, n,
                     lower_threshold, stats, stats_scratch, statistics, words, words_host, result, stream, record_rows=None):
diff --git a/levelsetfusion-python_amd/engine_slavcheva.py b/levelsetfusion-python_amd/engine_slavcheva.py
--- a/levelsetfusion-python_amd/engine_slavcheva.py
+++ b/levelsetfusion-python_amd/engine_slavcheva.py
@@ -111,6 +111,8 @@
         self.log = None
         self._fast = self._gradient_state = self._cumulative_state = self._sobolev_band = None
         self._g4_cache, self._cut_chunk_cache = None, (None, None)
+        self._list_capacity = {}
+        self._run_scratch = (None, None)
         self._exchange_every_iteration = False
         self._slab_restore = self._pending_halos = None
         self._comm_stream = self._events = self._plan_stream = self._no_face = None
```
